# mprib/caliscope

Hardware: AMD Instinct MI355X
Metric: observations/sec per LM iteration (higher is better)
Workload: dtype f64; 1 GPU; cfg4: 64 cams / 2000000 obs in total (200000 points / 2000000 obs on rank 0), extrinsics-only BA, linear loss; n_obs_total=2000000, params_per_camera=6, tolerances=ftol=xtol=gtol=1e-8 (reference defaults), sums=FP64 atomics (default)

## Files before the change

### caliscope_amd/build.py

```python

from __future__ import annotations

import os
import shutil
import subprocess
import sys
from pathlib import Path

HERE = Path(__file__).resolve().parent
CSRC = HERE / "csrc"
OUT = HERE / "libcaliscope_ba.so"
SOURCES = [CSRC / "cba_lib.hip", CSRC / "cba_solve.cpp", CSRC / "pose_lib.hip", CSRC / "scale_lib.hip", CSRC / "coverage_lib.hip", CSRC / "vertical_lib.hip", CSRC / "report_lib.hip", CSRC / "trajectory_lib.hip", CSRC / "covariance_lib.hip"]
DEPENDS = [CSRC / "cba_kernels.h", CSRC / "schur_plan.h", CSRC / "host_plan.h", CSRC / "wg_binding.h", CSRC / "ba_math.h", CSRC / "trf_math.h", CSRC / "pnp_math.h", CSRC / "epipolar_math.h", CSRC / "intrinsic_math.h", CSRC / "frame_select_math.h", CSRC / "scale_math.h", CSRC / "coverage_math.h", CSRC / "vertical_math.h", CSRC / "report_math.h", CSRC / "trajectory_math.h", CSRC / "covariance_math.h", CSRC / "device_call.h",
           HERE.parent / "include" / "caliscope_ba.h", HERE.parent / "include" / "caliscope_pose.h", HERE.parent / "include" / "caliscope_coverage.h", HERE.parent / "include" / "caliscope_vertical.h", HERE.parent / "include" / "caliscope_report.h", HERE.parent / "include" / "caliscope_trajectory.h", HERE.parent / "include" / "caliscope" / "uncertainty.h"]
ARCH = "gfx950"


def hipcc_path() -> str:
    for cand in (os.environ.get("HIPCC"), shutil.which("hipcc"), "/opt/rocm/bin/hipcc"):
        if cand and Path(cand).exists():
            return cand
    raise RuntimeError("hipcc not found (expected /opt/rocm/bin/hipcc)")


def needs_build() -> bool:
    if not OUT.exists():
        return True
    t = OUT.stat().st_mtime
    return any(p.stat().st_mtime > t for p in SOURCES + DEPENDS)


def source_digest() -> str:
    import hashlib

    h = hashlib.sha256()
    for path in sorted(SOURCES + DEPENDS, key=lambda q: q.name):
        h.update(path.name.encode())
        h.update(path.read_bytes())
    return h.hexdigest()


def built_digest(path: Path = OUT) -> str | None:
    import re

    m = re.search(rb"CBA_SOURCE_DIGEST=([0-9a-f]{64})", path.read_bytes())
    return m.group(1).decode() if m else None


def build(force: bool = False, verbose: bool = True) -> Path:
    if not force and not needs_build() and built_digest() == source_digest():
        return OUT
    cmd = [
        hipcc_path(), f"--offload-arch={ARCH}", "-O3", "-std=c++17", "-shared", "-fPIC", "-munsafe-fp-atomics",
        "-Wall", "-Wno-unused-function", f'-DCBA_SOURCE_DIGEST="{source_digest()}"', *map(str, SOURCES), "-o", str(OUT), "-pthread", "-lrccl",
        "-lrocprofiler-sdk-roctx",
    ]
    if verbose:
        print("[caliscope_amd.build]", " ".join(cmd), flush=True)
    subprocess.run(cmd, check=True, cwd=str(CSRC))
    return OUT


if __name__ == "__main__":
    build(force="--force" in sys.argv)
    print(OUT)
```

### caliscope_amd/csrc/cba_kernels.h

```cpp
#pragma once
#include <hip/hip_runtime.h>

#include "ba_math.h"
#include "trf_math.h"
#include "wg_binding.h"

namespace cba {

constexpr int BLOCK = 256;
constexpr int CHUNK = 256;
constexpr int WAVE = 64;

struct VecLayout {
  int ncp;
  int ncp_pad;
  int P;
  int Ppad;
  __host__ __device__ long total() const { return (long)ncp_pad + 3L * Ppad; }
};

__device__ __forceinline__ double wave_sum(double v) {
#pragma unroll
  for (int o = WAVE / 2; o > 0; o >>= 1) v += __shfl_down(v, o, WAVE);
  return v;
}
__device__ __forceinline__ double wave_max(double v) {
#pragma unroll
  for (int o = WAVE / 2; o > 0; o >>= 1) v = fmax(v, __shfl_down(v, o, WAVE));
  return v;
}
#ifdef CBA_PROFILING
constexpr int STAMP_SLOTS = 96, STAMP_BLOCKS = 1024, STAMP_WAVES = 16, STAMP_ROW = 1 + STAMP_WAVES;
__device__ long long* g_cba_stamps = nullptr;
struct StampScope {
  long long* row;
  __device__ __forceinline__ explicit StampScope(int slot) : row(nullptr) {
    long long* base = g_cba_stamps;
    const int b = (int)(blockIdx.y * gridDim.x + blockIdx.x);
    if (base && slot < STAMP_SLOTS && b < STAMP_BLOCKS) {
      row = base + ((long)slot * STAMP_BLOCKS + b) * STAMP_ROW;
      if (threadIdx.x == 0 && threadIdx.y == 0) row[0] = wall_clock64();
    }
  }
  __device__ __forceinline__ ~StampScope() {
    const int t = (int)(threadIdx.y * blockDim.x + threadIdx.x);
    if (row && (t & (WAVE - 1)) == 0 && t / WAVE < STAMP_WAVES) row[1 + t / WAVE] = wall_clock64();
  }
};
#define CBA_STAMP(slot) StampScope cba_stamp_scope_(slot)
#else
#define CBA_STAMP(slot) ((void)0)
#endif
enum StampId { ST_TPREP = 0, ST_PAIRS, ST_REG_REDUCE, ST_FINALIZE, ST_CHOL_APPLY, ST_BACKSUB, ST_STEP_CAM, ST_BUILD, ST_REDUCE_PUB, ST_SCALE_LIN, ST_JV,
               ST_SMALL_SOLVE, ST_CHOL_STEP  };

__device__ __forceinline__ double block_sum(double v, double* sh) {
  v = wave_sum(v);
  const int lane = threadIdx.x & (WAVE - 1), w = threadIdx.x / WAVE;
  __syncthreads();
  if (lane == 0) sh[w] = v;
  __syncthreads();
  double r = 0.0;
  if (threadIdx.x == 0)
    for (int i = 0; i < BLOCK / WAVE; ++i) r += sh[i];
  return r;
}
__device__ __forceinline__ double block_max(double v, double* sh) {
  v = wave_max(v);
  const int lane = threadIdx.x & (WAVE - 1), w = threadIdx.x / WAVE;
  __syncthreads();
  if (lane == 0) sh[w] = v;
  __syncthreads();
  double r = 0.0;
  if (threadIdx.x == 0)
    for (int i = 0; i < BLOCK / WAVE; ++i) r = fmax(r, sh[i]);
  return r;
}

__device__ __forceinline__ void lds_add(double* addr, double v) { unsafeAtomicAdd(addr, v); }

constexpr int CAMTAB_LIVE = 36;
constexpr int CAMTAB_LDS = CAMTAB_LIVE + 1;
struct ObsRec { double u, v; int cam, pt; };
__device__ __forceinline__ ObsRec load_obs(const double* __restrict__ obs_u, const double* __restrict__ obs_v,
                                           const int* __restrict__ obs_cam, const int* __restrict__ obs_pt, int i) {
  ObsRec r;
  r.u = obs_u[i]; r.v = obs_v[i]; r.cam = obs_cam[i]; r.pt = obs_pt[i];
  return r;
}

__device__ __forceinline__ void stage_camtab(double* sh_tab, const double* tab, int n_cams) {
  for (int i = threadIdx.x; i < n_cams * CAMTAB_LIVE; i += BLOCK)
    sh_tab[(i / CAMTAB_LIVE) * CAMTAB_LDS + (i % CAMTAB_LIVE)] = tab[(i / CAMTAB_LIVE) * CAMTAB_DOUBLES + (i % CAMTAB_LIVE)];
}
__device__ __forceinline__ const CamTab& cam_at(const double* sh_tab, int cam) {
  return *reinterpret_cast<const CamTab*>(sh_tab + cam * CAMTAB_LDS);
}
template <bool CAMG>
__device__ __forceinline__ const CamTab& cam_of(const double* sh_tab, const double* __restrict__ tab, int cam) {
  if constexpr (CAMG) return *reinterpret_cast<const CamTab*>(tab + (long)cam * CAMTAB_DOUBLES);
  else return cam_at(sh_tab, cam);
}

__global__ void k_cam_prep(const double* __restrict__ xvec, const double* __restrict__ cam_const,
                           const int* __restrict__ cam_model, const int* __restrict__ cam_np,
                           const int* __restrict__ cam_off, int n_cams, double* __restrict__ tab) {
  const int c = blockIdx.x * blockDim.x + threadIdx.x;
  if (c >= n_cams) return;
  double xc[MAX_NC];
  const int np = cam_np[c];
  for (int i = 0; i < MAX_NC; ++i) xc[i] = (i < np) ? xvec[cam_off[c] + i] : 0.0;
  CamTab t;
  cam_prepare(xc, cam_const + c * CAM_CONST_STRIDE, cam_model[c], np, &t, cam_off[c]);
  const double* src = reinterpret_cast<const double*>(&t);
  for (int i = 0; i < CAMTAB_DOUBLES; ++i) tab[c * CAMTAB_DOUBLES + i] = src[i];
}

__global__ void __launch_bounds__(BLOCK)
k_begin(const double* __restrict__ x0, double* __restrict__ x, double* __restrict__ x_new, double* __restrict__ sinv, double* __restrict__ cam_diag,
        int* __restrict__ flags, long total, int ncp_pad, const double* __restrict__ cam_const, const int* __restrict__ cam_model,
        const int* __restrict__ cam_np, const int* __restrict__ cam_off, int n_cams, double* __restrict__ tab) {
  const long t0 = (long)blockIdx.x * blockDim.x + threadIdx.x;
  for (long i = t0; i < total; i += (long)gridDim.x * blockDim.x) {
    const double v = x0[i];
    x[i] = v;
    if (x_new) x_new[i] = v;
    sinv[i] = 1.0;
    if (i < ncp_pad) cam_diag[i] = 0.0;
    if (i < 4) flags[i] = 0;
  }
  if (t0 < n_cams) {
    const int c = (int)t0;
    double xc[MAX_NC];
    const int np = cam_np[c];
    for (int i = 0; i < MAX_NC; ++i) xc[i] = (i < np) ? x0[cam_off[c] + i] : 0.0;
    CamTab t;
    cam_prepare(xc, cam_const + c * CAM_CONST_STRIDE, cam_model[c], np, &t, cam_off[c]);
    const double* src = reinterpret_cast<const double*>(&t);
    for (int i = 0; i < CAMTAB_DOUBLES; ++i) tab[c * CAMTAB_DOUBLES + i] = src[i];
  }
}

template <bool WRITE_R, bool CAMG = false>
__global__ void __launch_bounds__(BLOCK)
k_cost(const double* __restrict__ obs_u, const double* __restrict__ obs_v, const int* __restrict__ obs_cam,
       const int* __restrict__ obs_pt, long n_obs, const double* __restrict__ xvec, VecLayout lay,
       const double* __restrict__ tab, int n_cams, int loss, double f_scale, double* __restrict__ partial,
       int* __restrict__ flags, double* __restrict__ r_out, const int* __restrict__ order) {
  extern __shared__ __attribute__((aligned(16))) double sh[];
  double* sh_tab = sh;
  double* sh_red = sh + (CAMG ? 0 : n_cams * CAMTAB_LDS);
  if (!CAMG) stage_camtab(sh_tab, tab, n_cams);
  __syncthreads();
  const double* px = xvec + lay.ncp_pad;
  double acc = 0.0;
  bool bad = false;
  struct Rec { int cam, pt; double u, v; long o; };
  const long stride = (long)gridDim.x * BLOCK, last = n_obs - 1;
// ... 1724 lines not shown
    v = -sum;
  } else {
    v = -Sacc[(long)row * ncp + col];
  }
  if (same_cam) v += Upacked[param_cam[row] * UP::STRIDE + UP::idx(param_loc[row], param_loc[col])];
  if (row == col) v += lam * sinv[row] * sinv[row] + cam_diag[row];
  return v;
}
template <int NC>
__global__ void __launch_bounds__(256)
k_schur_finalize(const double* __restrict__ Sacc, const double* __restrict__ bacc,
                 const double* __restrict__ Upacked, const double* __restrict__ gvec,
                 const double* __restrict__ sinv, const int* __restrict__ param_cam,
                 const int* __restrict__ param_loc, int ncp, double lam, const double* __restrict__ lam_dev,
                 const double* __restrict__ cam_diag, double* __restrict__ S, double* __restrict__ rhs,
                 double* __restrict__ W, int ldw, const double* __restrict__ red = nullptr, int g = 0, long tile_elems = 0,
                 const int* __restrict__ group_cam_begin = nullptr, int b_width = 0) {
  CBA_STAMP(ST_FINALIZE);
  if (lam_dev) lam = *lam_dev;
  const long t = (long)blockIdx.x * blockDim.x + threadIdx.x;
  if (t >= (long)ncp * ncp) return;
  const int row = (int)(t / ncp), col = (int)(t % ncp);
  if (col < row) return;
  const double v = schur_entry<NC>(row, col, Sacc, Upacked, sinv, param_cam, param_loc, ncp, lam, cam_diag, red, g, tile_elems, group_cam_begin);
  if (row == col) {
    const double rv = -gvec[row] + b_entry(bacc, b_width, row);
    rhs[row] = rv;
    W[(long)ncp * ldw + row] = rv;
  }
  S[(long)row * ncp + col] = v;
  S[(long)col * ncp + row] = v;
  W[(long)row * ldw + col] = v;
  W[(long)col * ldw + row] = v;
}

template <int NC>
__global__ void __launch_bounds__(64 * REG_REDUCE_Y_MAX)
k_reg_finalize(TilePlan tp, const int* __restrict__ tile_wg_begin, const double* __restrict__ partial, const int* __restrict__ cam_off,
               const int* __restrict__ cam_np, int ncp, int n_tiles, int G, int ysplit, int fold_x, int rhs_x, int tile_x,
               const double* __restrict__ partial_b, int b_rows, int b_width,
               const double* __restrict__ Upacked, const double* __restrict__ gvec, const double* __restrict__ sinv, double lam,
               const double* __restrict__ lam_dev, const double* __restrict__ cam_diag, double* __restrict__ S, double* __restrict__ rhs,
               double* __restrict__ W, int ldw) {
  CBA_STAMP(ST_REG_REDUCE);
  using UP = UPack<NC>;
  constexpr int YM = REG_REDUCE_Y_MAX;
  __shared__ double sh[YM][64];
  const int tx = threadIdx.x, ty = threadIdx.y;
  const int g = tp.g, bsz = NC * NC;
  auto put = [&](int row, int col, double v) {
    S[(long)row * ncp + col] = v; S[(long)col * ncp + row] = v;
    W[(long)row * ldw + col] = v; W[(long)col * ldw + row] = v;
  };
  const int bid = (int)blockIdx.x;
  if (bid >= G * fold_x && bid < G * fold_x + rhs_x) {
    const int j = (bid - G * fold_x) * 64 + tx;
    sh[ty][tx] = (j < b_width) ? strided_sum(partial_b + j, b_width, 0, b_rows, ty, YM) : 0.0;
    __syncthreads();
    if (ty == 0 && j < ncp) {
      double tot = 0.0;
#pragma unroll
      for (int y = 0; y < YM; ++y) tot += sh[y][tx];
      const double rv = -gvec[j] + tot;
      rhs[j] = rv;
      W[(long)ncp * ldw + j] = rv;
    }
    return;
  }
  if (bid < G * fold_x) {
    if (lam_dev) lam = *lam_dev;
    const int ga = bid / fold_x, bx = bid % fold_x;
    const int t = ga * G - ga * (ga - 1) / 2;
    const int ca0 = tp.group_cam_begin[ga], na = tp.group_cam_begin[ga + 1] - ca0;
    const int q = bx * 64 + tx;
    const int cl = q / bsz, r = (q % bsz) / NC, c = (q % bsz) % NC;
    const bool live = q < g * bsz && cl < na && c >= r && c < cam_np[ca0 + min(cl, max(na - 1, 0))];
    constexpr int HMAX = kSchurRegMaxGroupK * (kSchurRegMaxGroupK + 1) / 2;
    __shared__ int sh_hoff[3][HMAX];
    const int cl_first = (bx * 64) / bsz;
    for (int e = ty * 64 + tx; e < 3 * HMAX; e += 64 * YM) {
      const int cam_l = cl_first + e / HMAX, h = e % HMAX, k = cam_l + h * max(na, 1);
      int off = 0;
      if (cam_l < na && k < g * (g + 1) / 2) {
        int li = (int)((sqrtf(8.0f * k + 1.0f) - 1.0f) * 0.5f);
        while (li * (li + 1) / 2 > k) --li;
        while ((li + 1) * (li + 2) / 2 <= k) ++li;
        off = (li * g + (k - li * (li + 1) / 2)) * bsz;
      }
      sh_hoff[e / HMAX][h] = off;
    }
    __syncthreads();
    double a[8] = {0.0, 0.0, 0.0, 0.0, 0.0, 0.0, 0.0, 0.0};
    const int w0 = tile_wg_begin[t] * tp.rep, R = tile_wg_begin[t + 1] * tp.rep - w0;
    if (live && R > 0) {
      const int H = (g * (g + 1) / 2 - cl + na - 1) / na;
      const int* hoff = sh_hoff[cl - cl_first];
      const double* base = partial + (long)w0 * tp.tile_elems + r * NC + c;
      int h = ty / R, w = ty % R;
      auto next = [&]() {
        const double* ptr = base + (long)w * tp.tile_elems + hoff[min(h, H - 1)];
        w += YM;
        while (w >= R) { w -= R; ++h; }
        return ptr;
      };
      const int total = H * R;
      int m = ty;
      for (; m + 7 * YM < total; m += 8 * YM) {
        const double* ptr[8];
#pragma unroll
        for (int q = 0; q < 8; ++q) ptr[q] = next();
#pragma unroll
        for (int q = 0; q < 8; ++q) a[q] += *ptr[q];
      }
      for (; m < total; m += YM) a[0] += *next();
    }
    sh[ty][tx] = ((a[0] + a[1]) + (a[2] + a[3])) + ((a[4] + a[5]) + (a[6] + a[7]));
    __syncthreads();
    if (ty != 0 || !live) return;
    double tot = 0.0;
#pragma unroll
    for (int y = 0; y < YM; ++y) tot += sh[y][tx];
    const int cam = ca0 + cl, row = cam_off[cam] + r, col = cam_off[cam] + c;
    double v = Upacked[cam * UP::STRIDE + UP::idx(r, c)] - tot;
    if (r == c) v += lam * sinv[row] * sinv[row] + cam_diag[row];
    put(row, col, v);
    return;
  }
  const int t = (bid - G * fold_x - rhs_x) / tile_x, bx = (bid - G * fold_x - rhs_x) % tile_x;
  const int ga = tp.tile_a[t], gb = tp.tile_b[t];
  const int ca0 = tp.group_cam_begin[ga], na = tp.group_cam_begin[ga + 1] - ca0;
  const int cb0 = tp.group_cam_begin[gb], nb = tp.group_cam_begin[gb + 1] - cb0;
  const int per = YM / ysplit, sub = ty / ysplit, yy = ty % ysplit;
  const int e = (bx * per + sub) * 64 + tx;
  const int w0 = tile_wg_begin[t] * tp.rep, w1 = tile_wg_begin[t + 1] * tp.rep;
  int row = -1, col = -1;
  if (e < g * g * bsz) {
    const int beta = e / bsz, rc = e % bsz;
    const int li = beta / g, lj = beta % g, r = rc / NC, c = rc % NC;
    if (!(ga == gb && lj <= li) && li < na && lj < nb && r < cam_np[ca0 + li] && c < cam_np[cb0 + lj]) {
      row = cam_off[ca0 + li] + r; col = cam_off[cb0 + lj] + c;
    }
  }
  sh[ty][tx] = (row >= 0) ? strided_sum(partial + e, tp.tile_elems, w0, w1, yy, ysplit) : 0.0;
  __syncthreads();
  if (yy != 0 || row < 0) return;
  double tot = 0.0;
  for (int y = 0; y < ysplit; y += 4) tot += (sh[ty + y][tx] + sh[ty + y + 1][tx]) + (sh[ty + y + 2][tx] + sh[ty + y + 3][tx]);
  put(row, col, -tot);
}

typedef double v4f64 __attribute__((ext_vector_type(4)));
constexpr int CHOL_THREADS = 512;

__device__ __forceinline__ void chol_rank_nb(const double* __restrict__ A, int rcA, const double* __restrict__ B, int rcB,
                                             int ldw, double (*red)[16][17], int wv, int lane) {
  if (wv >= 4) return;
  const int ti = wv >> 1, tj = wv & 1, lr = lane & 15, kq = 4 * (lane >> 4);
  const double* pa = A + (long)min(ti * 16 + lr, rcA - 1) * ldw + kq;
  const double* pb = B + (long)min(tj * 16 + lr, rcB - 1) * ldw + kq;
  double2 a[NB / 16][2], b[NB / 16][2];
#pragma unroll
  for (int s = 0; s < NB / 16; ++s)
#pragma unroll
    for (int h = 0; h < 2; ++h) {
      a[s][h] = *reinterpret_cast<const double2*>(pa + 16 * s + 2 * h);
      b[s][h] = *reinterpret_cast<const double2*>(pb + 16 * s + 2 * h);
    }
  v4f64 c = {0.0, 0.0, 0.0, 0.0};
#pragma unroll
  for (int s = 0; s < NB / 16; ++s)
#pragma unroll
    for (int h = 0; h < 2; ++h) {
      c = __builtin_amdgcn_mfma_f64_16x16x4f64(a[s][h].x, b[s][h].x, c, 0, 0, 0);
      c = __builtin_amdgcn_mfma_f64_16x16x4f64(a[s][h].y, b[s][h].y, c, 0, 0, 0);
    }
#pragma unroll
  for (int r = 0; r < 4; ++r) red[wv][(lane >> 4) + 4 * r][lr] = c[r];
}

__global__ void __launch_bounds__(CHOL_THREADS)
k_chol_step(double* __restrict__ W, int n, int ldw, int k, int* __restrict__ flags, long long* __restrict__ trace, double* __restrict__ Xinv,
            double* __restrict__ Tinv = nullptr) {
  CBA_STAMP(ST_CHOL_STEP + k + 1);
  __shared__ double sh_red[4][16][17];
  __shared__ double sh_U[NB][NB + 1], sh_X[NB][NB + 1], sh_D[2 * NB][NB + 1];
  __shared__ __attribute__((aligned(16))) double sh_L[NB][NB + 2];
  const int tid = threadIdx.x, wv = tid >> 6, lane = tid & 63;
  const int nbk = (n + NB - 1) / NB;
  constexpr int EPT = NB * NB / CHOL_THREADS, ISTEP = CHOL_THREADS / NB;
  const int j = tid & 31, i0 = tid >> 5;
  const int n_panel = (k < 0) ? 1 : nbk - k;
  const int n_trailing = (k < 1) ? 0 : (nbk - k - 1) * (nbk - k) / 2;

  if ((int)blockIdx.x >= n_panel + n_trailing) {
    const int t2 = blockIdx.x - n_panel - n_trailing;
    const int bi = k + t2 / k, bj = t2 % k, m = k - 1;
    const int ri = bi * NB, rci = min(NB, n - ri), rj = bj * NB, rcj = min(NB, n - rj);
    double* Tb = Tinv + (long)rj * ldw + ri;
    double old[EPT];
#pragma unroll
    for (int h = 0; h < EPT; ++h) {
      const int i = i0 + h * ISTEP;
      old[h] = (m != bj && i < rcj && j < rci) ? Tb[(long)i * ldw + j] : 0.0;
    }
    chol_rank_nb(Tinv + (long)rj * ldw + m * NB, rcj, W + (long)ri * ldw + m * NB, rci, ldw, sh_red, wv, lane);
    __syncthreads();
    if (bi != k) {
#pragma unroll
      for (int h = 0; h < EPT; ++h) {
        const int i = i0 + h * ISTEP;
        if (i < rcj && j < rci) Tb[(long)i * ldw + j] = old[h] + sh_red[(i >> 4) * 2 + (j >> 4)][i & 15][j & 15];
      }
      return;
    }
#pragma unroll
    for (int h = 0; h < EPT; ++h) {
      const int i = i0 + h * ISTEP;
      sh_U[i][j] = (i < rcj && j < rci) ? old[h] + sh_red[(i >> 4) * 2 + (j >> 4)][i & 15][j & 15] : 0.0;
      sh_L[i][j] = Xinv[(long)k * NB * NB + i * NB + j];
    }
    __syncthreads();
    if (wv < 4) {
      const int ti = wv >> 1, tj = wv & 1;
      v4f64 c = {0.0, 0.0, 0.0, 0.0};
#pragma unroll
      for (int t = 0; t < NB / 4; ++t) {
        const int q = 4 * t + (lane >> 4);
        c = __builtin_amdgcn_mfma_f64_16x16x4f64(sh_U[ti * 16 + (lane & 15)][q], sh_L[tj * 16 + (lane & 15)][q], c, 0, 0, 0);
      }
#pragma unroll
      for (int r = 0; r < 4; ++r) {
        const int i = ti * 16 + (lane >> 4) + 4 * r, jj = tj * 16 + (lane & 15);
        if (i < rcj && jj < rci) Tb[(long)i * ldw + jj] = -c[r];
      }
    }
    return;
  }

  if ((int)blockIdx.x >= n_panel) {
    int t = blockIdx.x - n_panel, bj = k + 1;
    while (t >= nbk - bj) { t -= nbk - bj; ++bj; }
    const int bi = bj + 1 + t;
    const int ri = (bi < nbk) ? bi * NB : n, rci = (bi < nbk) ? min(NB, n - ri) : 1;
    const int rj = bj * NB, rcj = min(NB, n - rj);
    const int m0 = (k - 1) * NB;
    double* Wi = W + (long)ri * ldw;
    double w_ij[EPT];
#pragma unroll
    for (int h = 0; h < EPT; ++h) {
      const int i = i0 + h * ISTEP;
      w_ij[h] = (i < rci && j < rcj) ? Wi[(long)i * ldw + rj + j] : 0.0;
    }
    chol_rank_nb(Wi + m0, rci, W + (long)rj * ldw + m0, rcj, ldw, sh_red, wv, lane);
    __syncthreads();
#pragma unroll
    for (int h = 0; h < EPT; ++h) {
      const int i = i0 + h * ISTEP;
      if (i < rci && j < rcj) Wi[(long)i * ldw + rj + j] = w_ij[h] - sh_red[(i >> 4) * 2 + (j >> 4)][i & 15][j & 15];
    }
    return;
  }

  const int b = k + 1 + blockIdx.x;
  const int rb = (b < nbk) ? b * NB : n;
  const int rc = (b < nbk) ? min(NB, n - rb) : 1;
  const bool has_diag = b < nbk;
  double* Wb = W + (long)rb * ldw;
  const bool stamp = trace != nullptr && blockIdx.x == 0 && tid == 0;
#define CHOL_STAMP(ph) do { if (stamp) trace[(k + 1) * 8 + (ph)] = wall_clock64(); } while (0)
  CHOL_STAMP(0);

  double d_ij[EPT], m_ij[EPT], l_ij[EPT];
#pragma unroll
  for (int h = 0; h < EPT; ++h) {
    const int i = i0 + h * ISTEP;
    d_ij[h] = (has_diag && i < rc && j < rc) ? Wb[(long)i * ldw + rb + j] : (i == j ? 1.0 : 0.0);
  }
  if (k < 0) {
#pragma unroll
    for (int h = 0; h < EPT; ++h) sh_D[i0 + h * ISTEP][j] = d_ij[h];
  } else {
    const int k0 = k * NB, nbp = min(NB, n - k0);
#pragma unroll
    for (int h = 0; h < EPT; ++h) {
      const int i = i0 + h * ISTEP;
      m_ij[h] = (i < rc && j < nbp) ? Wb[(long)i * ldw + k0 + j] : 0.0;
      l_ij[h] = Xinv[(long)k * NB * NB + i * NB + j];
    }

    CHOL_STAMP(1);
    if (k >= 1) chol_rank_nb(Wb + (k0 - NB), rc, W + (long)k0 * ldw + (k0 - NB), nbp, ldw, sh_red, wv, lane);
    __syncthreads();
    CHOL_STAMP(2);
#pragma unroll
    for (int h = 0; h < EPT; ++h) {
      const int i = i0 + h * ISTEP;
      const double upd = (k >= 1) ? sh_red[(i >> 4) * 2 + (j >> 4)][i & 15][j & 15] : 0.0;
      sh_U[i][j] = m_ij[h] - upd;
      sh_L[i][j] = l_ij[h];
    }
    __syncthreads();
    CHOL_STAMP(3);
    if (wv < 4) {
      const int ti = wv >> 1, tj = wv & 1;
      v4f64 c = {0.0, 0.0, 0.0, 0.0};
#pragma unroll
      for (int t = 0; t < NB / 4; ++t) {
        const int q = 4 * t + (lane >> 4);
        c = __builtin_amdgcn_mfma_f64_16x16x4f64(sh_U[ti * 16 + (lane & 15)][q], sh_L[tj * 16 + (lane & 15)][q], c, 0, 0, 0);
      }
#pragma unroll
      for (int r = 0; r < 4; ++r) {
        const int i = ti * 16 + (lane >> 4) + 4 * r, jj = tj * 16 + (lane & 15);
        sh_X[i][jj] = (jj < nbp && i < rc) ? c[r] : 0.0;
      }
    }
    __syncthreads();
#pragma unroll
    for (int h = 0; h < EPT; ++h) {
      const int i = i0 + h * ISTEP;
      if (i < rc && j < nbp) Wb[(long)i * ldw + k0 + j] = sh_X[i][j];
    }
    CHOL_STAMP(4);
    if (!has_diag) return;
    if (wv < 4) {
      const int ti = wv >> 1, tj = wv & 1;
      v4f64 c = {0.0, 0.0, 0.0, 0.0};
#pragma unroll
      for (int t = 0; t < NB / 4; ++t) {
        const int q = 4 * t + (lane >> 4);
        c = __builtin_amdgcn_mfma_f64_16x16x4f64(sh_X[ti * 16 + (lane & 15)][q], sh_X[tj * 16 + (lane & 15)][q], c, 0, 0, 0);
      }
#pragma unroll
      for (int r = 0; r < 4; ++r) sh_red[wv][(lane >> 4) + 4 * r][lane & 15] = c[r];
    }
    __syncthreads();
#pragma unroll
    for (int h = 0; h < EPT; ++h) {
      const int i = i0 + h * ISTEP;
      const double d_new = d_ij[h] - sh_red[(i >> 4) * 2 + (j >> 4)][i & 15][j & 15];
      if (b != k + 1) {
        if (i < rc && j < rc) Wb[(long)i * ldw + rb + j] = d_new;
      } else {
        sh_D[i][j] = (i < rc && j < rc) ? d_new : (i == j ? 1.0 : 0.0);
      }
    }
    if (b != k + 1) return;
  }
  __syncthreads();
  CHOL_STAMP(5);
  if (tid < WAVE) chol_factor_block(sh_D, rc, flags);
  __syncthreads();
  chol_factor_store(sh_D, rc, Wb + rb, ldw, Xinv + (long)(k + 1) * NB * NB, tid, CHOL_THREADS, Tinv ? Tinv + (long)rb * ldw + rb : nullptr);
  CHOL_STAMP(6);
#undef CHOL_STAMP
}

constexpr int SMALL_N = 96;
constexpr int SMALL_THREADS = 512;
constexpr int SMALL_LD = SMALL_N + 1;
template <int NC>
__global__ void __launch_bounds__(SMALL_THREADS)
k_small_solve(const double* __restrict__ Sacc, const double* __restrict__ bacc, const double* __restrict__ Upacked, const double* __restrict__ gvec,
              const double* __restrict__ sinv, const int* __restrict__ param_cam, const int* __restrict__ param_loc, int n, double lam,
              const double* __restrict__ lam_dev, const double* __restrict__ cam_diag, double* __restrict__ S, double* __restrict__ rhs,
              const double* __restrict__ red, int g, long tile_elems, const int* __restrict__ group_cam_begin, int* __restrict__ flags,
              double* __restrict__ out, int b_width) {
  CBA_STAMP(ST_SMALL_SOLVE);
  using UP = UPack<NC>;
  extern __shared__ __attribute__((aligned(16))) double sh[];
  double (*W)[SMALL_LD] = reinterpret_cast<double (*)[SMALL_LD]>(sh);
  double (*D)[NB + 1] = reinterpret_cast<double (*)[NB + 1]>(sh + (SMALL_N + 1) * SMALL_LD);
  double (*X)[NB][NB + 1] = reinterpret_cast<double (*)[NB][NB + 1]>(&D[2 * NB][0]);
  double* y = &X[(SMALL_N + NB - 1) / NB][0][0];
  if (lam_dev) lam = *lam_dev;
  const int tid = threadIdx.x, nbk = (n + NB - 1) / NB;
  int* pc = reinterpret_cast<int*>(y + SMALL_N);
  int* pl = pc + SMALL_N;
  for (int i = tid; i < n; i += SMALL_THREADS) {
    pc[i] = param_cam[i]; pl[i] = param_loc[i];
    const double rv = -gvec[i] + b_entry(bacc, b_width, i);
    rhs[i] = rv;
    W[n][i] = rv;
  }
  __syncthreads();
  for (int base = tid; base < n * n; base += 4 * SMALL_THREADS) {
    double v4[4];
    int r4[4], c4[4];
#pragma unroll
    for (int u = 0; u < 4; ++u) {
      const int t = base + u * SMALL_THREADS;
      const int row = min(t, n * n - 1) / n, col = min(t, n * n - 1) % n;
      const bool live = t < n * n && col > row && pc[row] != pc[col];
      r4[u] = live ? row : -1; c4[u] = col;
      v4[u] = -Sacc[(long)row * n + col];
    }
#pragma unroll
    for (int u = 0; u < 4; ++u) {
      if (r4[u] < 0) continue;
      S[(long)r4[u] * n + c4[u]] = v4[u]; S[(long)c4[u] * n + r4[u]] = v4[u];
      W[r4[u]][c4[u]] = v4[u]; W[c4[u]][r4[u]] = v4[u];
    }
  }
  for (int q = tid; q < n * NC; q += SMALL_THREADS) {
    const int row = q / NC, col = row - pl[row] + q % NC;
    if (col < row || col >= n || pc[col] != pc[row]) continue;
    const int cam = pc[row];
    double v;
    if (red) {
      const int ga = cam / g, ca0 = group_cam_begin[ga], na = group_cam_begin[ga + 1] - ca0;
      const double* src = red + (long)ga * tile_elems + pl[row] * NC + pl[col];
      double sum = 0.0;
      for (int k = cam - ca0; k < g * (g + 1) / 2; k += na) {
        int li = (int)((sqrtf(8.0f * k + 1.0f) - 1.0f) * 0.5f);
        while (li * (li + 1) / 2 > k) --li;
        while ((li + 1) * (li + 2) / 2 <= k) ++li;
        const int lj = k - li * (li + 1) / 2;
        sum += src[(long)(li * g + lj) * (NC * NC)];
      }
      v = -sum;
    } else {
      v = -Sacc[(long)row * n + col];
    }
    v += Upacked[cam * UP::STRIDE + UP::idx(pl[row], pl[col])];
    if (row == col) v += lam * sinv[row] * sinv[row] + cam_diag[row];
    S[(long)row * n + col] = v; S[(long)col * n + row] = v;
    W[row][col] = v; W[col][row] = v;
  }
  __syncthreads();
  for (int k = 0; k < nbk; ++k) {
    const int k0 = k * NB, nb = min(NB, n - k0);
    for (int e = tid; e < NB * NB; e += SMALL_THREADS) {
      const int i = e / NB, j = e % NB;
      D[i][j] = (i < nb && j < nb) ? W[k0 + max(i, j)][k0 + min(i, j)] : (i == j ? 1.0 : 0.0);
    }
    __syncthreads();
    if (tid < WAVE) chol_factor_block(D, nb, flags);
    __syncthreads();
    for (int e = tid; e < NB * NB; e += SMALL_THREADS) {
      const int i = e / NB, j = e % NB;
      if (i < nb && j <= i) W[k0 + i][k0 + j] = D[i][j];
      X[k][i][j] = D[NB + j][i];
    }
    __syncthreads();
    const int r_lo = k0 + nb, n_rows = n + 1 - r_lo;
    double acc4[(SMALL_N + 1) * NB / SMALL_THREADS + 1];
    {
      int q = 0;
      for (int e = tid; e < n_rows * NB; e += SMALL_THREADS, ++q) {
        const int r = r_lo + e / NB, j = e % NB;
        double a = 0.0;
        if (j < nb)
          for (int t = 0; t <= j; ++t) a = fma(W[r][k0 + t], X[k][j][t], a);
        acc4[q] = a;
      }
    }
    __syncthreads();
    {
      int q = 0;
      for (int e = tid; e < n_rows * NB; e += SMALL_THREADS, ++q) {
        const int r = r_lo + e / NB, j = e % NB;
        if (j < nb) W[r][k0 + j] = acc4[q];
      }
    }
    __syncthreads();
    const int m = n - r_lo;
    for (int e = tid; e < (m + 1) * m; e += SMALL_THREADS) {
      const int i = r_lo + e / m, j = r_lo + e % m;
      if (j > i) continue;
      double a = W[i][j];
      for (int t = 0; t < nb; ++t) a = fma(-W[i][k0 + t], W[j][k0 + t], a);
      W[i][j] = a;
    }
    __syncthreads();
  }
  for (int i = tid; i < n; i += SMALL_THREADS) y[i] = W[n][i];
  __syncthreads();
  for (int k = nbk - 1; k >= 0; --k) {
    const int k0 = k * NB, nb = min(NB, n - k0);
    double xv = 0.0;
    if (tid < nb) {
      for (int t = tid; t < nb; ++t) xv = fma(X[k][t][tid], y[k0 + t], xv);
    }
    __syncthreads();
    if (tid < nb) { y[k0 + tid] = xv; out[k0 + tid] = xv; }
    __syncthreads();
    for (int i = tid; i < k0; i += SMALL_THREADS) {
      double a = y[i];
      for (int t = 0; t < nb; ++t) a = fma(-W[k0 + t][i], y[k0 + t], a);
      y[i] = a;
    }
    __syncthreads();
  }
}

constexpr int APPLY_THREADS = 512;
__global__ void __launch_bounds__(APPLY_THREADS)
k_chol_apply(const double* __restrict__ Tinv, const double* __restrict__ W, int n, int ldw, double* __restrict__ out) {
  CBA_STAMP(ST_CHOL_APPLY);
  extern __shared__ __attribute__((aligned(16))) double y[];
  const int tid = threadIdx.x;
  for (int i = tid; i < n; i += APPLY_THREADS) y[i] = W[(long)n * ldw + i];
  __syncthreads();
  const int r = tid >> 4, cl = tid & 15, row = blockIdx.x * NB + r;
// ... 1451 lines not shown
```

### caliscope_amd/csrc/cba_lib.hip

```cpp
#include <hip/hip_runtime.h>

#include <algorithm>
#include <atomic>
#include <chrono>
#include <cmath>
#include <condition_variable>
#include <cstdarg>
#include <cstdio>
#include <cstdlib>
#include <cstring>
#include <map>
#include <mutex>
#include <shared_mutex>
#include <memory>
#include <string>
#include <type_traits>
#include <thread>
#include <utility>
#include <vector>

#include <rccl/rccl.h>
#include <rocprofiler-sdk-roctx/roctx.h>

#include "../../include/caliscope_ba.h"
#include "cba_kernels.h"
#include "schur_plan.h"
#include "host_plan.h"
#include "wg_binding.h"

using namespace cba;

#ifndef CBA_SOURCE_DIGEST
#define CBA_SOURCE_DIGEST "unknown"
#endif
extern "C" __attribute__((used, visibility("hidden"))) const char cba_source_digest_marker[] = "CBA_SOURCE_DIGEST=" CBA_SOURCE_DIGEST;

static thread_local std::string g_last_error;

static int fail(int code, const char* fmt, ...) {
  char buf[1024];
  va_list ap;
  va_start(ap, fmt);
  vsnprintf(buf, sizeof(buf), fmt, ap);
  va_end(ap);
  g_last_error = buf;
  return code;
}

#define HIPCHK(expr)                                                                                   \
  do {                                                                                                 \
    hipError_t _e = (expr);                                                                            \
    if (_e != hipSuccess)                                                                              \
      return fail(CBA_ERR_HIP, "%s failed: %s (%s:%d)", #expr, hipGetErrorString(_e), __FILE__, __LINE__); \
  } while (0)

enum TimerId {
  T_CAM_PREP = 0, T_COST, T_BUILD, T_BUILD_REDUCE, T_SCALE_SCALARS, T_JV, T_SCHUR, T_SCHUR_REDUCE, T_CHOLESKY,
  T_BACKSUB, T_VECTOR, T_SCHUR_PAIRS, T_EXCHANGE, T_COUNT
};
static const char* kTimerNames[T_COUNT] = {
    "cam_prep", "cost", "build", "build_reduce", "scale_scalars", "jv", "schur", "schur_reduce_finalize",
    "cholesky_solve", "backsub", "vector_ops", "schur_pairs", "exchange"};

struct EventPair { hipEvent_t a, b; };
struct cba_group;

constexpr int JV_ROWS = 2048, CON_ROWS = 1024, PARTIAL4_ROWS = JV_ROWS + CON_ROWS;

struct cba_problem {
  int device = 0;
  hipStream_t stream = nullptr;
  int C = 0, P = 0, ncp = 0, nct = 6;
  long N = 0;
  VecLayout lay{};
  int n_chunks = 0, grid = 0, max_obs_per_point = 0;
  int G = 1, gsz = 1, n_tiles = 1, n_tile_chunks = 0, tile_grid = 0;
  int cus = 256;
  double plan_lane_util = 0.0;
  long tile_stream_len = 0, n_pairs = 0;
  TilePlan tp{};
  int* tile_wg_begin = nullptr;
  int loss = 0;
  double f_scale = 1.0;
  long device_bytes = 0;
  double *obs_u = nullptr, *obs_v = nullptr;
  int *obs_cam = nullptr, *obs_pt = nullptr, *pt_start = nullptr, *chunk_start = nullptr, *order = nullptr;
  int* chunk_pts = nullptr;
  double* cam_const = nullptr;
  int *cam_model = nullptr, *cam_np = nullptr, *cam_off = nullptr, *param_cam = nullptr, *param_loc = nullptr;
  double *tab = nullptr, *tab_new = nullptr;
  double *x0 = nullptr, *x = nullptr, *x_new = nullptr, *g = nullptr, *s = nullptr, *sinv = nullptr, *v1 = nullptr, *v2 = nullptr;
  double *V = nullptr, *Upacked = nullptr;
  double *partial = nullptr, *partial4 = nullptr, *partial1 = nullptr;
  long partial_width = 0;
  bool want_chol_trace = false;
  long long* chol_trace = nullptr;
  int ldw = 0;
  double *Sacc = nullptr, *S = nullptr, *Lbuf = nullptr, *rhs = nullptr, *red = nullptr, *Trec = nullptr, *partial_b = nullptr;
  CsPlan cs{};
  bool tab_global = false;
  int det_m = 0;
  DetPlan det{nullptr, nullptr};
  double* tri = nullptr;
  double* Xinv = nullptr;
  double* Tinv = nullptr;
  bool fuse_reg_finalize = true;
  double* scal = nullptr;
  double* xbuf = nullptr;
  double *sinv_state_c = nullptr, *cam_diag = nullptr, *cam_over1 = nullptr, *cam_over2 = nullptr;
  bool cam_scaled = false, cam_state_saved = false;
  double *fz = nullptr, *V2 = nullptr, *g2 = nullptr, *U2 = nullptr, *partial4b = nullptr;
  bool eval_only = false;
  bool peer_needs_primitives = false;
  bool have_build = false;
  bool trial_built = false;
  bool cost_pending = false;
  double cost_x = 0.0;
  double trial_cost = 0.0;
  int grid_backsub = 1;
  int jv_grid = 0;
  bool has_fragments = false;
  bool backsub_rec = false;
  int n_heavy = 0; int* heavy_pts = nullptr; int* heavy_frag = nullptr; double* heavy_W = nullptr;
  std::vector<int> h_heavy_pts;
  ConPlan con{};
  int con_grid = 0;
  int n_con_orphan = 0; int* con_orphan = nullptr;
  int* flags = nullptr;
  double* h_scal = nullptr;
  int* h_flags = nullptr;
  double* d_hscal = nullptr;
  double *h_cam = nullptr, *d_hcam = nullptr;
  double *h_bcam = nullptr, *d_hbcam = nullptr;
  double *lb_dev = nullptr, *ub_dev = nullptr, *sinv_state_c2 = nullptr, *cam_diag2 = nullptr;
  bool bounds_on = false;
  unsigned long long publish_seq = 0;
  bool spin_wait = true;
  int* d_hflags = nullptr;
  bool first_scale = true;
  double* sinv2 = nullptr;
  bool spec_enqueued = false, spec_valid = false;
  int spec_rows_jv = 0;
  bool spec_skip = true, tol_set = false, last_trial_hint = false;
  double ftol = 0.0, xtol = 0.0;
  int* spec_word = nullptr;
  bool spec_jv_enqueued = false;
  bool spec_jv_dropped = false;
  bool spec_scale_ready = false;
  long spec_jv_skipped = 0;
  unsigned long long gnorm_seq = 0;
  bool gnorm_mailed = false;
  bool lf_pending = false;
  LinFin lf{};
  bool have_x0 = false;
  std::vector<int> h_tile_wg_begin;
  struct PlanTask* plan_task = nullptr;
  int reg_reduce_y = 4;
  int plan_max_blocks = 0;
  size_t partial_capacity = 0;
  bool plan_is_cheap = false;
  int plan_error = 0;
  bool schur_clock = false;
  long long* stamps = nullptr;
  bool begun = false, linearized = false, stepped = false, have_trial = false;
  double gh_sq = 0.0;
  std::vector<int> h_cam_off, h_cam_np;
  double* h_vec = nullptr;
  size_t h_vec_doubles = 0;
  hipEvent_t h_vec_sent = nullptr;
  bool h_vec_in_flight = false;
  bool timers_on = false;
  std::vector<EventPair> pending[T_COUNT];
  std::vector<EventPair> free_events;
  double t_ms[T_COUNT] = {0};
  long t_calls[T_COUNT] = {0};
  std::vector<void*> allocs;
  std::vector<size_t> alloc_bytes;
  size_t mail_doubles = 0;
  char* arena_cur = nullptr; size_t arena_left = 0, arena_next = (size_t)4 << 20;
  char* up_stage = nullptr; size_t up_cap = 0, up_used = 0;
  std::atomic<ncclComm_t> comm{nullptr};
  std::atomic<bool> comm_aborted{false};
  cba_group* group = nullptr;
  int rank = 0, world = 1;
  unsigned long long group_generation = 0;
  bool sharded() const { return comm.load() != nullptr || group != nullptr || comm_aborted.load(); }
  bool small_solve_on = true;
  bool one_workgroup_solve() const { return ncp <= SMALL_N && small_solve_on && !sharded() && !chol_trace; }
};

constexpr size_t kPoolChunk = (size_t)4 << 20;
constexpr size_t kPoolKeep = 4;
constexpr size_t kPoolStagingMax = (size_t)8 << 20;
struct DevicePool {
  std::vector<void*> chunks;
  std::vector<hipStream_t> streams;
  std::vector<std::pair<double*, size_t>> mail;
  std::vector<std::pair<double*, size_t>> staging;
  std::vector<char*> upstage;
};
constexpr size_t kUpStage = (size_t)256 << 10, kUpStageMax = (size_t)64 << 10;
static std::mutex g_pool_mu;
static std::map<int, DevicePool> g_pool;

template <typename T>
static int dev_alloc(cba_problem* p, T** out, size_t count) {
  const size_t bytes = (std::max<size_t>(count, 1) * sizeof(T) + 255) & ~(size_t)255;
  if (bytes > p->arena_left) {
    const size_t chunk = std::max(bytes, p->arena_next);
    void* ptr = nullptr;
    if (chunk == kPoolChunk) {
      std::lock_guard<std::mutex> lock(g_pool_mu);
      DevicePool& pool = g_pool[p->device];
      if (!pool.chunks.empty()) { ptr = pool.chunks.back(); pool.chunks.pop_back(); }
    }
    if (!ptr) HIPCHK(hipMalloc(&ptr, chunk));
    p->allocs.push_back(ptr);
    p->alloc_bytes.push_back(chunk);
    if (bytes >= p->arena_next) {
      p->device_bytes += (long)bytes;
      *out = static_cast<T*>(ptr);
      return CBA_OK;
    }
    p->arena_cur = static_cast<char*>(ptr);
    p->arena_left = chunk;
    p->arena_next = std::min<size_t>(p->arena_next * 2, (size_t)256 << 20);
  }
  *out = reinterpret_cast<T*>(p->arena_cur);
  p->arena_cur += bytes;
  p->arena_left -= bytes;
  p->device_bytes += (long)bytes;
  return CBA_OK;
}
template <typename T>
static int dev_upload(cba_problem* p, T** out, const T* h, size_t count) {
  int rc = dev_alloc(p, out, count);
  if (rc) return rc;
  const size_t bytes = count * sizeof(T);
  if (bytes && p->up_stage && p->stream && bytes <= kUpStageMax && p->up_used + bytes <= p->up_cap) {
    std::memcpy(p->up_stage + p->up_used, h, bytes);
    HIPCHK(hipMemcpyAsync(*out, p->up_stage + p->up_used, bytes, hipMemcpyHostToDevice, p->stream));
    p->up_used += (bytes + 63) & ~(size_t)63;
  } else if (bytes) {
    HIPCHK(hipMemcpy(*out, h, bytes, hipMemcpyHostToDevice));
  }
  return CBA_OK;
}
template <typename T, typename V>
static int dev_upload(cba_problem* p, T** out, const V& h) {
  static_assert(std::is_same<typename std::remove_cv<typename std::remove_pointer<decltype(h.data())>::type>::type, T>::value, "element type");
  return dev_upload(p, out, h.data(), h.size());
}
template <typename T>
static int dev_zeros(cba_problem* p, T** out, size_t count) {
  int rc = dev_alloc(p, out, count);
  if (rc) return rc;
  HIPCHK(hipMemsetAsync(*out, 0, count * sizeof(T), p->stream));
  return CBA_OK;
// ... 716 lines not shown
        p->grid_backsub = std::max(1, std::min(p->n_chunks, p->cus * resident_per_cu(k_backsub_rec<NC, true>, lds_backsub_rec<NC>(p), 2)));
    }
  }
  {
    int per_cu = p->tab_global ? resident_per_cu(k_jv<NC, 1, true>, lds_jv(p, 1), 2) : resident_per_cu(k_jv<NC, 1>, lds_jv(p, 1), 2);
    if (const char* e = std::getenv("CBA_JV_WGS")) per_cu = std::max(1, std::min(std::atoi(e), 8));
    p->jv_grid = (int)std::max<long>(1, std::min<long>((p->N + BLOCK - 1) / BLOCK, (long)p->cus * per_cu));
    p->jv_grid = std::min(p->jv_grid, JV_ROWS);
  }
  if (p->n_heavy && (rc = allow_lds(k_heavy_schur<NC>, (size_t)p->ncp * 3 * sizeof(double) + (size_t)p->ncp * sizeof(int)))) return rc;
  if ((rc = allow_lds(k_chol_apply, (size_t)p->ncp * 8))) return rc;
  if ((rc = allow_lds(k_step_cam, (size_t)p->lay.ncp_pad * 8))) return rc;
  if (p->one_workgroup_solve() && (rc = allow_lds(k_small_solve<NC>, kSmallSolveLds))) return rc;
  return CBA_OK;
}


static void start_plan_task(cba_problem* p, const cba_options* opt, int n_cus, const int* hcam, const int* hps) {
  constexpr long kTwoStageObs = 500000;
  const char* plan_env = std::getenv("CBA_PLAN");
  bool plan_two_stage = p->N >= kTwoStageObs;
  if (plan_env && std::strcmp(plan_env, "swap") == 0) plan_two_stage = true;
  if (plan_env && (std::strcmp(plan_env, "full") == 0 || std::strcmp(plan_env, "cheap") == 0)) plan_two_stage = false;
  if ((opt && opt->deterministic) || p->schur_clock) plan_two_stage = false;
  Reg2Params prm = (p->nct == 9) ? reg2_params<9, Reg3Cfg<9>>(p) : reg2_params<6, Reg3Cfg<6>>(p);
  if (plan_env) prm.cheap = std::strcmp(plan_env, "cheap") == 0;
  p->plan_task = new PlanTask();
  {
    const int cus0 = n_cus > 0 ? n_cus : 256;
    const size_t tile_lds = (p->nct == 9) ? Reg3Cfg<9>::LDS_BYTES : Reg3Cfg<6>::LDS_BYTES;
    const int per_cu = std::min(std::max<int>(1, (int)((160 * 1024) / tile_lds)), (p->nct == 9) ? RegCfg<9>::PER_CU : RegCfg<6>::PER_CU);
    const int mb0 = (opt && opt->max_blocks > 0) ? opt->max_blocks : 2 * cus0;
    p->plan_max_blocks = std::min(cus0 * per_cu, std::max(mb0, cus0));
  }
  p->plan_task->start(prm, hcam, hps, plan_two_stage, p);
}

static int open_stream_and_mailbox(cba_problem* p, const MailLayout& mail) {
  {
    std::lock_guard<std::mutex> lock(g_pool_mu);
    DevicePool& pool = g_pool[p->device];
    if (!pool.streams.empty()) { p->stream = pool.streams.back(); pool.streams.pop_back(); }
    for (size_t i = 0; i < pool.mail.size(); ++i)
      if (pool.mail[i].second >= mail.total) {
        p->h_scal = pool.mail[i].first; p->mail_doubles = pool.mail[i].second;
        pool.mail.erase(pool.mail.begin() + (long)i);
        break;
      }
  }
  if (!p->stream) HIPCHK(hipStreamCreateWithFlags(&p->stream, hipStreamNonBlocking));
  if (!p->h_scal) {
    p->mail_doubles = std::max<size_t>(mail.total, MailLayout(96).total);
    HIPCHK(hipHostMalloc((void**)&p->h_scal, p->mail_doubles * sizeof(double), hipHostMallocMapped));
  }
  HIPCHK(hipHostGetDevicePointer((void**)&p->d_hscal, p->h_scal, 0));
  p->h_cam = p->h_scal + mail.cam; p->d_hcam = p->d_hscal + mail.cam;
  p->h_flags = reinterpret_cast<int*>(p->h_scal + mail.flags); p->d_hflags = reinterpret_cast<int*>(p->d_hscal + mail.flags);
  p->h_bcam = p->h_scal + mail.bcam; p->d_hbcam = p->d_hscal + mail.bcam;
  std::memset(p->h_scal, 0, mail.total * sizeof(double));
  return CBA_OK;
}

#define TRYS(e) do { const int rc_ = (e); if (rc_) return rc_; } while (0)

static int upload_observations(cba_problem* p, const double* obs_uv, const SortedObs& obs, const PointTables& tabs) {
  TRYS(dev_upload(p, &p->obs_cam, obs.cam)); TRYS(dev_upload(p, &p->obs_pt, obs.pt));
  TRYS(dev_upload(p, &p->order, obs.order)); TRYS(dev_upload(p, &p->pt_start, tabs.pt_start)); TRYS(dev_upload(p, &p->chunk_start, tabs.chunk_start));
  double* uv_raw = nullptr;
  TRYS(dev_upload(p, &uv_raw, obs_uv, (size_t)2 * p->N)); TRYS(dev_alloc(p, &p->obs_u, (size_t)p->N)); TRYS(dev_alloc(p, &p->obs_v, (size_t)p->N));
  hipLaunchKernelGGL(k_gather_uv, dim3((int)std::min<long>((p->N + 255) / 256, 2048)), dim3(256), 0, p->stream, (const double*)uv_raw, (const int*)p->order, p->N, p->obs_u, p->obs_v);
  return CBA_OK;
}

static int upload_det_plan(cba_problem* p, const HostDetPlan& plan) {
  unsigned char* dperm = nullptr; unsigned short* dcst = nullptr;
  TRYS(dev_upload(p, &dperm, plan.perm)); TRYS(dev_upload(p, &dcst, plan.cst));
  p->det_m = plan.det_m;
  p->det = DetPlan{dperm, dcst};
  return CBA_OK;
}

static int upload_cs_plan(cba_problem* p, const HostCsPlan& plan) {
  double *dcu = nullptr, *dcv = nullptr;
  int *dcc = nullptr, *dcp = nullptr, *dso = nullptr, *dp0 = nullptr, *dnp = nullptr, *dperm = nullptr;
  TRYS(dev_upload(p, &dperm, plan.cperm));
  TRYS(dev_alloc(p, &dcu, (size_t)p->N)); TRYS(dev_alloc(p, &dcv, (size_t)p->N)); TRYS(dev_alloc(p, &dcc, (size_t)p->N)); TRYS(dev_alloc(p, &dcp, (size_t)p->N));
  TRYS(dev_upload(p, &dso, plan.sc_obs)); TRYS(dev_upload(p, &dp0, plan.sc_p0)); TRYS(dev_upload(p, &dnp, plan.sc_np));
  hipLaunchKernelGGL(k_cs_fill, dim3(plan.n_sc), dim3(256), 0, p->stream, (const int*)dperm, (const int*)dso, (const int*)dp0, (const double*)p->obs_u, (const double*)p->obs_v,
                     (const int*)p->obs_cam, (const int*)p->obs_pt, dcu, dcv, dcc, dcp);
  p->cs = CsPlan{dcu, dcv, dcc, dcp, dso, dp0, dnp, plan.n_sc, plan.pmax};
  return CBA_OK;
}

static int upload_cameras(cba_problem* p, const double* cam_const, const CameraLayout& cams, const PointTables& tabs) {
  if (p->n_heavy) {
    TRYS(dev_upload(p, &p->heavy_pts, tabs.heavy)); TRYS(dev_upload(p, &p->heavy_frag, tabs.heavy_frag));
    TRYS(dev_alloc(p, &p->heavy_W, (size_t)p->n_heavy * p->ncp * 3));
  }
  TRYS(dev_upload(p, &p->cam_const, cam_const, (size_t)p->C * 12));
  TRYS(dev_upload(p, &p->cam_model, cams.model)); TRYS(dev_upload(p, &p->cam_np, cams.np)); TRYS(dev_upload(p, &p->cam_off, cams.off));
  TRYS(dev_upload(p, &p->param_cam, cams.param_cam)); TRYS(dev_upload(p, &p->param_loc, cams.param_loc));
  return CBA_OK;
}

static int alloc_vectors(cba_problem* p) {
  TRYS(dev_alloc(p, &p->tab, (size_t)p->C * CAMTAB_DOUBLES)); TRYS(dev_alloc(p, &p->tab_new, (size_t)p->C * CAMTAB_DOUBLES));
  for (double** v : {&p->x0, &p->x, &p->x_new, &p->g, &p->s, &p->sinv, &p->v1, &p->v2, &p->sinv2}) TRYS(dev_zeros(p, v, (size_t)p->lay.total()));
  for (double** v : {&p->sinv_state_c, &p->cam_diag, &p->cam_over1, &p->cam_over2, &p->lb_dev, &p->ub_dev, &p->sinv_state_c2, &p->cam_diag2})
    TRYS(dev_zeros(p, v, (size_t)p->lay.ncp_pad));
  TRYS(dev_zeros(p, &p->V, (size_t)6 * p->lay.Ppad));
  const int ustride = (p->nct == 9) ? UPack<9>::STRIDE : UPack<6>::STRIDE;
  TRYS(dev_alloc(p, &p->Upacked, (size_t)p->C * ustride + 128));
  return CBA_OK;
}

static int install_first_plan(cba_problem* p, bool plan_timing) {
  PlanTask& task = *p->plan_task;
  const auto t_wait = std::chrono::steady_clock::now();
  task.wait_stage(task.two_stage ? 1 : 2);
  if (plan_timing) {
    fprintf(stderr, "  plan: %s took %.3f s on its own threads, started before the uploads; waited %.3f s for it\n", task.two_stage ? "the cheap plan" : "dealt streams and codes",
            task.two_stage ? task.seconds_cheap : task.seconds, std::chrono::duration<double>(std::chrono::steady_clock::now() - t_wait).count());
    const Reg2Plan& made = task.two_stage ? task.cheap : task.plan;
    fprintf(stderr, "  plan: its phases: point runs %.4f s, jobs %.4f s, concatenation %.4f s (%.0f MB)\n", made.seconds_runs, made.seconds_jobs, made.seconds_concat,
            (made.obs.size() + made.codes.size()) * 4e-6);
  }
  if (task.two_stage ? task.rc_cheap : task.rc)
    return fail(CBA_ERR_UNSUPPORTED, "a world point has more observations inside one camera-group tile than a chunk of the pair plan holds (%d records)",
                (p->nct == 9) ? Reg3Cfg<9>::SCHUNK : Reg3Cfg<6>::SCHUNK);
  const int rc = install_reg2_plan(p, task.two_stage ? task.cheap : task.plan, task.prm);
  p->plan_is_cheap = task.two_stage || task.prm.cheap;
  return rc;
}

static int alloc_solver_buffers(cba_problem* p) {
  const int ncp = p->ncp, nct = p->nct;
  const long tot = p->lay.total();
  const int ustride = (nct == 9) ? UPack<9>::STRIDE : UPack<6>::STRIDE;
  const long w_build = (long)p->C * ustride;
  p->partial_width = w_build;
  p->partial_capacity = (size_t)std::max<long>((long)p->grid * w_build, (long)(p->tile_grid + p->tile_grid / 8 + 1) * std::max(p->tp.rep, 1) * p->tp.tile_elems);
  TRYS(dev_alloc(p, &p->partial, p->partial_capacity));
  TRYS(dev_alloc(p, &p->partial4, (size_t)PARTIAL4_ROWS * 4)); TRYS(dev_alloc(p, &p->partial1, (size_t)2048)); TRYS(dev_alloc(p, &p->partial4b, (size_t)2048 * 4));
  TRYS(dev_zeros(p, &p->Sacc, (size_t)ncp * ncp + (size_t)B_SLICES * p->lay.ncp_pad));
  TRYS(dev_alloc(p, &p->tri, (size_t)ncp * (ncp + 1) / 2 + p->lay.ncp_pad));
  if (!p->eval_only) {
    TRYS(dev_alloc(p, &p->red, (size_t)p->G * p->tp.tile_elems));
    TRYS(dev_alloc(p, &p->Trec, (size_t)std::max<long>(p->N, 1) * ((nct == 9) ? SchurRec<9>::HREC : SchurRec<6>::HREC)));
    TRYS(dev_alloc(p, &p->partial_b, (size_t)p->grid * p->lay.ncp_pad));
  }
  TRYS(dev_alloc(p, &p->S, (size_t)ncp * ncp)); p->ldw = (ncp + 3) & ~3;
  if (p->want_chol_trace) TRYS(dev_alloc(p, &p->chol_trace, (size_t)((ncp + NB - 1) / NB + 2) * 8));
  TRYS(dev_alloc(p, &p->Lbuf, (size_t)(ncp + 1) * p->ldw));
  TRYS(dev_alloc(p, &p->Xinv, (size_t)((ncp + NB - 1) / NB + 1) * NB * NB));
  TRYS(dev_zeros(p, &p->Tinv, (size_t)ncp * p->ldw));
  TRYS(dev_alloc(p, &p->rhs, (size_t)p->lay.ncp_pad));
  TRYS(dev_zeros(p, &p->scal, 64)); TRYS(dev_zeros(p, &p->flags, 8)); TRYS(dev_alloc(p, &p->xbuf, 128));
  p->spec_word = p->flags + 4;
  TRYS(dev_alloc(p, &p->fz, 8)); TRYS(dev_zeros(p, &p->V2, (size_t)6 * p->lay.Ppad)); TRYS(dev_zeros(p, &p->g2, (size_t)tot));
  TRYS(dev_alloc(p, &p->U2, (size_t)p->C * ustride + 128));
  return CBA_OK;
}

static int open_staging(cba_problem* p) {
  const size_t tot = (size_t)p->lay.total();
  {
    std::lock_guard<std::mutex> lock(g_pool_mu);
    DevicePool& pool = g_pool[p->device];
    for (size_t i = 0; i < pool.staging.size(); ++i)
      if (pool.staging[i].second >= tot && pool.staging[i].second <= 4 * tot + 4096) {
        p->h_vec = pool.staging[i].first; p->h_vec_doubles = pool.staging[i].second;
        pool.staging.erase(pool.staging.begin() + (long)i);
        break;
      }
  }
  HIPCHK(hipEventCreateWithFlags(&p->h_vec_sent, hipEventDisableTiming));
  if (!p->h_vec) {
    p->h_vec_doubles = tot;
    HIPCHK(hipHostMalloc((void**)&p->h_vec, p->h_vec_doubles * sizeof(double), hipHostMallocDefault));
  }
  return CBA_OK;
}
static int device_synchronize() { HIPCHK(hipDeviceSynchronize()); return CBA_OK; }
#undef TRYS

extern "C" {

int cba_create(const cba_problem_desc* d, const cba_options* opt, cba_problem** out) {
  if (!d || !out) return fail(CBA_ERR_INVALID, "cba_create: null argument");
  *out = nullptr;
  if (const int rc = validate_problem_desc(fail, d)) return rc;
  const double t_enter = std::chrono::duration<double>(std::chrono::steady_clock::now().time_since_epoch()).count();
  int ndev = 0;
  if (hipGetDeviceCount(&ndev) != hipSuccess || ndev <= 0)
    return fail(CBA_ERR_NO_DEVICE, "no HIP device available: the MI355X engine has no CPU fallback");
  int dev = (opt && opt->device_id >= 0) ? opt->device_id : 0;
  if (!(opt && opt->device_id >= 0)) (void)hipGetDevice(&dev);
  if (dev >= ndev) return fail(CBA_ERR_INVALID, "device %d requested, %d available", dev, ndev);
  HIPCHK(hipSetDevice(dev));
  int n_cus = 0;
  if (hipDeviceGetAttribute(&n_cus, hipDeviceAttributeMultiprocessorCount, dev) != hipSuccess) n_cus = 0;

  cba_problem* p = new cba_problem();
  p->device = dev;
  p->C = d->n_cams; p->P = d->n_points; p->N = d->n_obs;
  p->loss = d->loss; p->f_scale = d->f_scale;
  if (const char* e = std::getenv("CBA_REG_FINALIZE")) p->fuse_reg_finalize = e[0] != '0';
  if (const char* e = std::getenv("CBA_SPEC_SKIP")) p->spec_skip = e[0] != '0';
  if (const char* e = std::getenv("CBA_SMALL_SOLVE")) p->small_solve_on = e[0] != '0';
#ifdef CBA_PROFILING
  p->schur_clock = std::getenv("CBA_SCHUR_CLOCK") != nullptr;
  p->want_chol_trace = std::getenv("CBA_CHOL_TRACE") != nullptr;
  if (std::getenv("CBA_STAMPS")) {
    const size_t n = (size_t)STAMP_SLOTS * STAMP_BLOCKS * STAMP_ROW;
    if (hipMalloc((void**)&p->stamps, n * sizeof(long long)) == hipSuccess) {
      (void)hipMemset(p->stamps, 0, n * sizeof(long long));
      (void)hipMemcpyToSymbol(HIP_SYMBOL(g_cba_stamps), &p->stamps, sizeof(p->stamps));
    }
  }
#endif
  int rc = CBA_OK;
#define TRY(e) do { rc = (e); if (rc) { cba_destroy(p); return rc; } } while (0)
  const bool deterministic = opt && opt->deterministic;

  CameraLayout cams;
  TRY(camera_layout(fail, d, cams));
  const int ncp = cams.ncp, nct = cams.nct;
  p->ncp = ncp; p->nct = nct;
  p->h_cam_off = cams.off; p->h_cam_np = cams.np;
  p->lay.ncp = ncp; p->lay.ncp_pad = cams.ncp_pad;
  p->lay.P = p->P; p->lay.Ppad = (p->P + 31) / 32 * 32;

  const bool plan_timing = plan_timing_on();
  auto t_now = []() { return std::chrono::duration<double>(std::chrono::steady_clock::now().time_since_epoch()).count(); };
  double t_mark = t_now();
  auto lap = [&](const char* what) { if (plan_timing) { const double t = t_now(); fprintf(stderr, "cba_create: %-28s %.6f s\n", what, t - t_mark); t_mark = t; } };
  SortedObs obs;
  PointTables tabs;
  {
    HostVec<int64_t> order(p->N), pstart((size_t)p->P + 1), cstart((size_t)p->N + 2);
    const int64_t nch = cba_host_plan(p->P, p->N, d->obs_pt, d->obs_cam, p->C, CHUNK, order.data(), pstart.data(), cstart.data());
    if (nch < 0) TRY((int)nch);
    p->n_chunks = (int)nch;
    lap("sort by point, chunk table");
    gather_sorted(p->N, d->obs_cam, d->obs_pt, order.data(), obs);
    TRY(point_tables(fail, p->P, pstart.data(), nch, cstart.data(), obs.pt.data(), CHUNK, HEAVY_OBS, tabs));
  }
  p->max_obs_per_point = tabs.max_obs_per_point;
  p->n_heavy = (int)tabs.heavy.size();
  p->h_heavy_pts = tabs.heavy;
  p->has_fragments = tabs.has_fragments;
  p->eval_only = opt && opt->evaluation_only != 0;
  choose_schur_groups(p);
  if (!p->eval_only) start_plan_task(p, opt, n_cus, obs.cam.data(), tabs.pt_start.data());

  TRY(open_stream_and_mailbox(p, MailLayout(ncp)));
  const int cus = n_cus > 0 ? n_cus : 256;
  p->cus = cus;
  const int max_blocks = (opt && opt->max_blocks > 0) ? opt->max_blocks : 2 * cus;
  p->grid = std::max(1, std::min(p->n_chunks, max_blocks));
  p->grid_backsub = std::max(1, std::min(p->n_chunks, 2 * cus));
  if (const char* e = std::getenv("CBA_BACKSUB_WGS")) p->grid_backsub = std::max(1, std::min(p->n_chunks, std::min(std::max(std::atoi(e), 1), 8) * cus));

  lap("reorder on host");
  upload_stage_acquire(p);
  TRY(upload_observations(p, d->obs_uv, obs, tabs));
  if (deterministic) {
    HostDetPlan det;
    TRY(det_plan(fail, p->C, nct, p->n_chunks, tabs.chunk_start.data(), obs.cam.data(), CHUNK, DET_ROUND, BLOCK, det));
    TRY(upload_det_plan(p, det));
  }
  TRY(dev_upload(p, &p->chunk_pts, tabs.chunk_pts));
  {
    const char* cs_env = std::getenv("CBA_BUILD_CS");
    HostCsPlan cs;
    cs_plan(!(cs_env && cs_env[0] == '0'), deterministic, p->C, p->N, p->n_chunks, tabs.chunk_start.data(), tabs.chunk_pts.data(), obs.cam.data(), p->grid,
            (nct == 9) ? 4096 : 2048, CHUNK, CS_MAX_PTS, cs);
    if (cs.n_sc) TRY(upload_cs_plan(p, cs));
  }
  TRY(upload_cameras(p, d->cam_const, cams, tabs));
  lap("upload observations");
  TRY(alloc_vectors(p));
  lap("allocate vectors");
  if (nct == 9) TRY(configure_kernels<9>(p)); else TRY(configure_kernels<6>(p));
  lap("reorder, upload, allocate");
  if (!p->eval_only) TRY(install_first_plan(p, plan_timing));
  lap("Schur plan (streams, pairs, upload)");
  TRY(alloc_solver_buffers(p));
  TRY(open_staging(p));
  lap("solver buffers");
  TRY(device_synchronize());
#undef TRY
  upload_stage_release(p);
  lap("device synchronize");
  if (p->plan_task) {
    if (p->plan_task->two_stage) {
      p->plan_task->hcam_keep = std::move(obs.cam);
      p->plan_task->hps_keep = std::move(tabs.pt_start);
    } else {
      drop_plan_task(p);
    }
  }
  if (plan_timing) fprintf(stderr, "cba_create: %.3f s in total\n", t_now() - t_enter);
  *out = p;
  return CBA_OK;
}

static int maybe_swap_plan(cba_problem* p, bool wait);

int cba_plan_wait(cba_problem* p) {
  if (!p) return fail(CBA_ERR_INVALID, "cba_plan_wait: null problem");
  HIPCHK(hipSetDevice(p->device));
  return maybe_swap_plan(p, true);
}

int cba_set_loss(cba_problem* p, int32_t loss, double f_scale) {
  if (!p) return fail(CBA_ERR_INVALID, "cba_set_loss: null problem");
  if (loss < CBA_LOSS_LINEAR || loss > CBA_LOSS_ARCTAN) return fail(CBA_ERR_INVALID, "cba_set_loss: unknown loss %d", loss);
  if (loss != CBA_LOSS_LINEAR && !(f_scale > 0.0)) return fail(CBA_ERR_INVALID, "cba_set_loss: f_scale must be positive");
  p->loss = loss; p->f_scale = f_scale;
  p->have_build = false;
  p->spec_valid = false; p->spec_enqueued = false; p->spec_scale_ready = false;
  return CBA_OK;
}

int cba_get_info(cba_problem* p, cba_info* o) {
  if (!p || !o) return fail(CBA_ERR_INVALID, "null argument");
  o->n_cams = p->C; o->n_points = p->P; o->n_cam_params = p->ncp; o->n_params = p->ncp + 3 * p->P; o->n_obs = p->N;
  o->n_chunks = p->n_chunks; o->grid_blocks = p->grid;
  o->plan_state = !p->plan_is_cheap ? 0 : (p->plan_task ? 1 : 2); o->plan_error = p->plan_error;
  o->schur_groups = p->G; o->schur_tiles = p->n_tiles; o->schur_grid = p->tile_grid; o->schur_stream_len = p->tile_stream_len; o->schur_pairs = p->n_pairs;
  o->max_obs_per_point = p->max_obs_per_point; o->device_bytes = p->device_bytes; o->n_heavy_points = p->n_heavy;
  {
    const bool cs = p->cs.n_sc && !p->det_m && !p->n_heavy;
    const bool camg = cs ? (p->nct == 6 ? build_cs_camg<6>(p) : build_cs_camg<9>(p)) : (p->nct == 6 ? build_camg<6>(p) : build_camg<9>(p));
    const bool uglob = cs && (p->nct == 6 ? build_cs_uglob<6>(p) : build_cs_uglob<9>(p));
    o->build_camg = (camg ? 1 : 0) | (p->tab_global ? 2 : 0) | (cs ? 4 : 0) | (uglob ? 8 : 0) | (p->backsub_rec ? 16 : 0) |
                    (p->con.n_con && p->con.small ? 32 : 0) | (p->one_workgroup_solve() ? 64 : 0);
  }
  o->spec_jv_skipped = p->spec_jv_skipped;
  return CBA_OK;
}

int cba_enable_timers(cba_problem* p, int32_t on) { if (!p) return fail(CBA_ERR_INVALID, "null"); p->timers_on = on != 0; return CBA_OK; }
int cba_reset_timers(cba_problem* p) {
  if (!p) return fail(CBA_ERR_INVALID, "null");
  (void)hipSetDevice(p->device);
  drain_timers(p);
  for (int t = 0; t < T_COUNT; ++t) { p->t_ms[t] = 0; p->t_calls[t] = 0; }
  return CBA_OK;
}
int cba_get_timers(cba_problem* p, double* ms, int64_t* calls) {
  if (!p) return fail(CBA_ERR_INVALID, "null");
  (void)hipSetDevice(p->device);
  drain_timers(p);
  for (int t = 0; t < T_COUNT; ++t) { if (ms) ms[t] = p->t_ms[t]; if (calls) calls[t] = p->t_calls[t]; }
  return CBA_OK;
}

}
// ... 101 lines not shown
      if (pub)
        hipLaunchKernelGGL(k_reduce_rows_pub, dim3((w + 63) / 64 + 1), dim3(64, REDUCE_RY), 0, p->stream, (const double*)p->partial, u_rows, w, Upacked, g,
                           (const int*)p->cam_off, (const int*)p->cam_np, (int)UPack<NC>::STRIDE, (int)UPack<NC>::TRI, *pub);
      else
        hipLaunchKernelGGL(k_reduce_rows, dim3((w + 63) / 64), dim3(64, REDUCE_RY), 0, p->stream, p->partial, u_rows, w, Upacked, g,
                           (const int*)p->cam_off, (const int*)p->cam_np, (int)UPack<NC>::STRIDE, (int)UPack<NC>::TRI);
      return CBA_OK;
    }
    hipLaunchKernelGGL(k_reduce_rows, dim3((w + 63) / 64), dim3(64, REDUCE_RY), 0, p->stream, p->partial, u_rows, w, Upacked,
                       (double*)nullptr, (const int*)nullptr, (const int*)nullptr, 1, 0);
    int rho_rows = p->grid;
    if (p->con.n_con) {
      HIPCHK(hipMemsetAsync(p->con.cdiag, 0, (size_t)3 * p->lay.Ppad * sizeof(double), p->stream));
      if (p->n_con_orphan)
        hipLaunchKernelGGL(k_zero_heavy, dim3((p->n_con_orphan + 63) / 64), dim3(64), 0, p->stream, (const int*)p->con_orphan, p->n_con_orphan, p->lay,
                           g + p->lay.ncp_pad, 3, (double*)nullptr, 0);
      hipLaunchKernelGGL(k_con_eval<true>, dim3(p->con_grid), dim3(BLOCK), 0, p->stream, p->con, xvec, p->lay, p->loss, p->f_scale, g,
                         p->partial1 + p->grid, p->flags, (double*)nullptr);
      rho_rows += p->con_grid;
    }
    hipLaunchKernelGGL(k_reduce_narrow<false>, dim3(1), dim3(BLOCK), 0, p->stream, p->partial1, rho_rows, 1, p->scal + cost_slot);
    if (defer_exchange) return CBA_OK;
    int rc = allreduce_sum(p, Upacked, (size_t)w);
    if (rc) return rc;
    hipLaunchKernelGGL((k_unpack_camera_grad<NC>), dim3((p->C * NC + 255) / 256), dim3(256), 0, p->stream, Upacked,
                       p->cam_off, p->cam_np, p->C, g);
  }
  return CBA_OK;
}

template <int NC>
static int run_build(cba_problem* p) { return run_build_into<NC>(p, p->x, p->tab, p->V, p->g, p->Upacked, 8, nullptr, false, false, 3); }

template <int NC>
static int run_jv(cba_problem* p, int nv, int* rows_out = nullptr, const double* xvec = nullptr, const double* tab = nullptr, const SpecSkip& skip = SpecSkip{}) {
  ScopedTimer t(p, T_JV);
  if (!xvec) { xvec = p->x; tab = p->tab; }
  const int grid = nv == 1 ? p->jv_grid : (int)std::min<long>((p->N + BLOCK - 1) / BLOCK, 1024);
  const int con_rows = p->con.n_con ? p->con_grid : 0;
  if (grid + con_rows > PARTIAL4_ROWS)
    return fail(CBA_ERR_UNSUPPORTED, "run_jv: %d rows of k_jv and %d of k_con_jv exceed the %d rows of partial4", grid, con_rows, PARTIAL4_ROWS);
  auto launch_jv = [&](auto kernel) {
    hipLaunchKernelGGL(kernel, dim3(grid), dim3(BLOCK), lds_jv(p, nv), p->stream, p->obs_u, p->obs_v, p->obs_cam, p->obs_pt,
                       p->N, xvec, p->lay, tab, p->cam_off, p->C, p->loss, p->f_scale, p->v1, p->v2, p->partial4, skip);
  };
  if (nv == 1) { if (p->tab_global) launch_jv(k_jv<NC, 1, true>); else launch_jv(k_jv<NC, 1>); }
  else { if (p->tab_global) launch_jv(k_jv<NC, 2, true>); else launch_jv(k_jv<NC, 2>); }
  int rows = grid;
  if (con_rows) {
    if (nv == 1) hipLaunchKernelGGL(k_con_jv<1>, dim3(p->con_grid), dim3(BLOCK), 0, p->stream, p->con, p->lay, p->v1, p->v2, p->partial4 + 4 * grid);
    else hipLaunchKernelGGL(k_con_jv<2>, dim3(p->con_grid), dim3(BLOCK), 0, p->stream, p->con, p->lay, p->v1, p->v2, p->partial4 + 4 * grid);
    rows += con_rows;
  }
  if (rows_out) { *rows_out = rows; return CBA_OK; }
  hipLaunchKernelGGL(k_reduce_narrow<false>, dim3(1), dim3(BLOCK), 0, p->stream, p->partial4, rows, 4, p->scal + 12);
  return CBA_OK;
}

template <int NC>
static int run_lin_chain(cba_problem* p, bool scalars = true, bool compact = false, double radius = 0.0, bool defer_finish = false) {
  RoctxRange range("cba:linearize");
  p->spec_scale_ready = false; p->gnorm_mailed = false;
  if (!p->have_build) {
    int rcb = run_build<NC>(p);
    if (rcb) return rcb;
    p->cost_pending = true;
    p->have_build = true;
    p->spec_valid = false;
  }
  if (compact && p->spec_valid) {
    p->spec_valid = false;
    if (defer_finish) {
      p->lf = LinFin{p->partial4b, p->partial1, p->partial4, vec_grid(p->lay.total()), p->spec_rows_jv, radius, p->scal, p->fz};
      p->lf_pending = true;
      return CBA_OK;
    }
    ScopedTimer t(p, T_SCALE_SCALARS);
    hipLaunchKernelGGL(k_lin_finish, dim3(1), dim3(BLOCK), 0, p->stream, p->partial4b, p->partial1, vec_grid(p->lay.total()), p->partial4, p->spec_rows_jv, radius,
                       p->scal, p->fz);
    return CBA_OK;
  }
  p->spec_valid = false;
  const long tot = p->lay.total();
  const int vg = vec_grid(tot);
  const bool bnd = defer_finish && p->bounds_on;
  if (bnd && !p->first_scale && !p->cam_scaled)
    HIPCHK(hipMemcpyAsync(p->sinv_state_c, p->sinv, (size_t)p->lay.ncp_pad * sizeof(double), hipMemcpyDeviceToDevice, p->stream));
  if (p->cam_scaled && !bnd)
    HIPCHK(hipMemcpyAsync(p->sinv, p->sinv_state_c, (size_t)p->lay.ncp_pad * sizeof(double), hipMemcpyDeviceToDevice, p->stream));
  p->cam_state_saved = false;
  {
    ScopedTimer t(p, T_SCALE_SCALARS);
    if (compact) {
      const BoundArgs ba = bnd ? BoundArgs{p->lb_dev, p->ub_dev, p->sinv_state_c, p->sinv_state_c, p->cam_diag} : BoundArgs{};
      if (bnd) p->cam_scaled = true;
      auto launch_sl = [&](auto kernel) {
        hipLaunchKernelGGL(kernel, dim3(vg), dim3(BLOCK), 0, p->stream, p->Upacked, p->V, p->param_cam, p->param_loc, p->lay,
                           p->first_scale ? 1 : 0, p->sinv, p->con.n_con ? (const double*)p->con.cdiag : (const double*)nullptr, p->x, p->g, p->v1,
                           p->partial4b, p->partial1, (const double*)nullptr, ba);
      };
      if (bnd) launch_sl(k_scale_lin<NC, true>); else launch_sl(k_scale_lin<NC, false>);
      p->first_scale = false;
      int rows_jv = 0;
      int rcj = run_jv<NC>(p, 1, &rows_jv);
      if (rcj) return rcj;
      if (defer_finish) {
        p->lf = LinFin{p->partial4b, p->partial1, p->partial4, vg, rows_jv, radius, p->scal, p->fz};
        p->lf_pending = true;
        return CBA_OK;
      }
      hipLaunchKernelGGL(k_lin_finish, dim3(1), dim3(BLOCK), 0, p->stream, p->partial4b, p->partial1, vg, p->partial4, rows_jv, radius,
                         p->scal, p->fz);
      return CBA_OK;
    }
    hipLaunchKernelGGL((k_scale_update<NC>), dim3(vg), dim3(BLOCK), 0, p->stream, p->Upacked, p->V, p->param_cam, p->param_loc,
                       p->lay, p->first_scale ? 1 : 0, p->sinv, p->con.n_con ? (const double*)p->con.cdiag : (const double*)nullptr);
    p->first_scale = false;
    if (!scalars) return exchange(p, SLOT(8), false);
    hipLaunchKernelGGL(k_lin_scalars, dim3(vg), dim3(BLOCK), 0, p->stream, p->x, p->g, p->sinv, tot, p->lay.ncp_pad,
                       p->rank == 0 ? 1 : 0, 0, p->v1, p->partial4, p->partial1);
    hipLaunchKernelGGL(k_reduce_narrow<false>, dim3(1), dim3(BLOCK), 0, p->stream, p->partial4, vg, 4, p->scal + 0);
    hipLaunchKernelGGL(k_reduce_narrow<true>, dim3(1), dim3(BLOCK), 0, p->stream, p->partial1, vg, 1, p->scal + 4);
  }
  {
    int rcj = run_jv<NC>(p, 1);
    if (rcj) return rcj;
  }
  return exchange(p, SLOT(0) | SLOT(1) | SLOT(2) | SLOT(3) | SLOT(8) | SLOT(12) | SLOT(13) | SLOT(14) | SLOT(15), true);
}

static void read_linearization(cba_problem* p, cba_linearization* out) {
  if (p->cost_pending) { p->cost_x = p->h_flags[3] ? NAN : 0.5 * p->h_scal[8]; p->cost_pending = false; }
  p->gh_sq = p->h_scal[0];
  out->gh_sq = p->h_scal[0];
  out->x_scaled_norm = std::sqrt(p->h_scal[1]);
  out->x_norm = std::sqrt(p->h_scal[2]);
  out->g_norm_inf = p->h_scal[4];
  out->cost = p->cost_x;
  out->jg_sq = p->h_scal[12];
}

template <int NC>
static int run_linearize(cba_problem* p, cba_linearization* out) {
  int rc = run_lin_chain<NC>(p, true, !p->sharded(), 1.0);
  if (rc) return rc;
  rc = sync_scalars(p, 16);
  if (rc) return rc;
  read_linearization(p, out);
  return CBA_OK;
}

namespace cba {
__attribute__((visibility("hidden"))) void enqueue_chol_factor(double* W, int n, int ldw, int* flags, long long* trace, double* Xinv, double* Tinv,
                                                               hipStream_t stream) {
  const int nbk = (n + NB - 1) / NB;
  for (int k = -1; k < nbk; ++k) {
    const int n_panel = k < 0 ? 1 : nbk - k;
    const int x = nbk - k - 1, n_trailing = k < 1 ? 0 : x * (x + 1) / 2;
    const int n_inverse = (k >= 1) ? (nbk - k) * k : 0;
    hipLaunchKernelGGL(k_chol_step, dim3(n_panel + n_trailing + n_inverse), dim3(CHOL_THREADS), 0, stream, W, n, ldw, k, flags, trace, Xinv, Tinv);
  }
}
}

static int enqueue_cholesky(cba_problem* p) {
  const int n = p->ncp, nbk = (n + NB - 1) / NB;
  enqueue_chol_factor(p->Lbuf, n, p->ldw, p->flags, p->chol_trace, p->Xinv, p->Tinv, p->stream);
  hipLaunchKernelGGL(k_chol_apply, dim3(nbk), dim3(APPLY_THREADS), (size_t)n * 8, p->stream, (const double*)p->Tinv, (const double*)p->Lbuf, n, p->ldw, p->s);
  return CBA_OK;
}

static int run_cholesky(cba_problem* p) {
#ifdef CBA_PROFILING
  if (p->chol_trace) {
    const int nbk = (p->ncp + NB - 1) / NB;
    HIPCHK(hipMemsetAsync(p->chol_trace, 0, (size_t)(nbk + 2) * 8 * sizeof(long long), p->stream));
    int rc = enqueue_cholesky(p);
    if (rc) return rc;
    std::vector<long long> h((size_t)(nbk + 2) * 8);
    HIPCHK(hipMemcpyAsync(h.data(), p->chol_trace, h.size() * sizeof(long long), hipMemcpyDeviceToHost, p->stream));
    HIPCHK(hipStreamSynchronize(p->stream));
    for (int s = 0; s <= nbk; ++s) {
      fprintf(stderr, "chol step %2d:", s - 1);
      for (int ph = 1; ph < 7; ++ph)
        if (h[s * 8 + ph] && h[s * 8 + ph - 1]) fprintf(stderr, " ph%d %6.2f us", ph, (h[s * 8 + ph] - h[s * 8 + ph - 1]) * 0.01); else if (h[s * 8 + ph]) fprintf(stderr, " ph%d (%6.2f)", ph, (h[s * 8 + ph] - h[s * 8]) * 0.01);
      if (s < nbk && h[(s + 1) * 8] && h[s * 8]) fprintf(stderr, "  | to next step start %6.2f us", (h[(s + 1) * 8] - h[s * 8]) * 0.01);
      fprintf(stderr, "\n");
    }
    return CBA_OK;
  }
#endif
  ScopedTimer t(p, T_CHOLESKY);
  return enqueue_cholesky(p);
}

static int run_step_scalars(cba_problem* p, bool formula_w, bool compact = false) {
  ScopedTimer t(p, T_VECTOR);
  const long tot = p->lay.total();
  const int vg = vec_grid(tot);
  const long first = (p->rank == 0) ? 0 : p->lay.ncp_pad;
  if (compact && first == 0 && tot <= STEP_SMALL_MAX) {
    hipLaunchKernelGGL(k_step_small, dim3(1), dim3(STEP_SMALL_THREADS), 0, p->stream, p->g, p->sinv, p->s, tot, p->scal, (const int*)p->flags, p->fz);
    return CBA_OK;
  }
  hipLaunchKernelGGL(k_step_scalars, dim3(vg), dim3(BLOCK), 0, p->stream, p->g, p->sinv, p->s, tot, first, p->partial4);
  if (compact) {
    hipLaunchKernelGGL(k_step_finish, dim3(1), dim3(BLOCK), 0, p->stream, p->partial4, vg, p->scal, (const int*)p->flags, p->fz);
    return CBA_OK;
  }
  hipLaunchKernelGGL(k_reduce_narrow<false>, dim3(1), dim3(BLOCK), 0, p->stream, p->partial4, vg, 4, p->scal + 16);
  if (formula_w) return exchange(p, SLOT(16) | SLOT(17), false);
  int rcv = allreduce_sum(p, p->scal + 16, 2);
  if (rcv) return rcv;
  hipLaunchKernelGGL(k_w_scalar, dim3(vg), dim3(BLOCK), 0, p->stream, p->g, p->sinv, p->s, tot, first, p->scal + 17, p->gh_sq,
                     (const double*)nullptr, p->partial1);
  hipLaunchKernelGGL(k_reduce_narrow<false>, dim3(1), dim3(BLOCK), 0, p->stream, p->partial1, vg, 1, p->scal + 20);
  return exchange(p, SLOT(20), false);
}

static int maybe_swap_plan(cba_problem* p, bool wait) {
  PlanTask* task = p->plan_task;
  if (!task) return CBA_OK;
  if (wait) task->wait_stage(2);
  if (task->stage.load(std::memory_order_acquire) < 2) return CBA_OK;
  int rc = CBA_OK;
  if (task->rc != 0 && task->two_stage) {
    p->plan_error = task->rc;
    fprintf(stderr, "caliscope_ba: the balanced Schur plan could not be built (error %d, %.3f s on its thread): the handle keeps the quick plan\n", task->rc, task->seconds);
    if (wait) rc = fail(task->rc, "cba_plan_wait: the balanced Schur plan could not be built in the background (error %d); the handle keeps the quick plan", task->rc);
  }
  if (task->rc == 0) {
    const size_t need = (size_t)task->install.tile_grid * std::max(task->install.tp.rep, 1) * task->install.tp.tile_elems;
    if (need > p->partial_capacity) {
      rc = dev_alloc(p, &p->partial, need);
      if (!rc) p->partial_capacity = need;
    }
    if (!rc) {
      apply_install(p, task->install);
      p->plan_is_cheap = false;
      if (plan_timing_on()) fprintf(stderr, "  plan: the dealt plan (%.3f s on its own threads, upload included) swapped in\n", task->seconds);
    }
  }
  drop_plan_task(p);
  return rc;
}

#ifdef CBA_PROFILING
template <int NC>
static int run_pairs_clocked(cba_problem* p) {
  if constexpr (NC != 6) return fail(CBA_ERR_UNSUPPORTED, "CBA_SCHUR_CLOCK: six-parameter cameras only");
  else {
    const int nw = Reg3Cfg<6>::NWAVES;
    const size_t n = (size_t)p->tile_grid * nw * 8;
    long long* d = nullptr;
    if (hipMalloc((void**)&d, n * sizeof(long long)) != hipSuccess) return fail(CBA_ERR_HIP, "debug buffer");
    (void)hipMemsetAsync(d, 0, n * sizeof(long long), p->stream);
    if (raise_lds_ceiling((const void*)k_schur_reg3_clk<6, 1, 2>, Reg3Cfg<6>::LDS_BYTES)) return CBA_ERR_HIP;
    hipLaunchKernelGGL((k_schur_reg3_clk<6, 1, 2>), dim3(p->tile_grid), dim3(Reg3Cfg<6>::LAUNCH_THREADS), Reg3Cfg<6>::LDS_BYTES, p->stream, p->tp, p->Trec, p->partial, d, (const double*)p->tab);
    std::vector<long long> h(n);
    (void)hipMemcpyAsync(h.data(), d, n * sizeof(long long), hipMemcpyDeviceToHost, p->stream);
    (void)hipStreamSynchronize(p->stream);
    (void)hipFree(d);
    static const char* names[4] = {"wait for loads", "barrier", "issue", "pairs"};
    auto report = [&](const char* who, auto pick) {
      double sum[8] = {0}, tmax = 0.0;
      size_t waves = 0;
      for (size_t w = 0; w < n / 8; ++w) {
        if (!h[w * 8 + 4] || !pick(w / nw)) continue;
        ++waves;
        for (int k = 0; k < 7; ++k) sum[k] += (double)h[w * 8 + k];
        tmax = std::max(tmax, (double)h[w * 8 + 6]);
      }
      const double wv = (double)std::max<size_t>(waves, 1);
      fprintf(stderr, "%s phases, mean clocks per wave (%zu waves, %.1f trips, %.1f pair iterations each):", who, waves, sum[4] / wv, sum[5] / wv);
      for (int k = 0; k < 4; ++k) fprintf(stderr, "  %s %.0f", names[k], sum[k] / wv);
      fprintf(stderr, "  | in-loop total %.0f, wave lifetime mean %.0f max %.0f\n", (sum[0] + sum[1] + sum[2] + sum[3]) / wv, sum[6] / wv, tmax);
    };
    report("k_schur_reg3", [](size_t) { return true; });
    return CBA_OK;
  }
}
#endif

template <int NC>
static int run_newton_chain(cba_problem* p, double lam, const double* lam_dev, bool compact = false) {
  const int ncp = p->ncp;
  if (p->plan_task) {
    const int rcs = maybe_swap_plan(p, false);
    if (rcs) return rcs;
  }
  RoctxRange range("cba:damped_step");
  {
    RoctxRange r2("cba:schur");
    ScopedTimer t(p, T_SCHUR);
    {
      const bool linf = p->lf_pending;
      p->lf_pending = false;
      auto launch_tprep = [&](auto kernel) {
        hipLaunchKernelGGL(kernel, dim3(p->grid), dim3(BLOCK), lds_tprep<NC>(p), p->stream, p->obs_u, p->obs_v, p->obs_cam, p->obs_pt,
                           p->chunk_start, p->n_chunks, p->x, p->lay, p->tab, p->cam_off, p->C, p->loss, p->f_scale, lam, lam_dev, p->V, p->g,
                           p->sinv, p->Trec, p->partial_b, p->flags, p->det, linf ? p->lf : LinFin{});
      };
      switch (p->det_m) {
        case 3: launch_tprep(k_tprep<NC, 3>); break;
        case 5: launch_tprep(k_tprep<NC, 5>); break;
        case 8: launch_tprep(k_tprep<NC, 8>); break;
        case 16: { if constexpr (NC == 6) launch_tprep(k_tprep<NC, 16>); } break;
        default:
          if (linf) { if (p->tab_global) launch_tprep(k_tprep<NC, 0, true, true>); else launch_tprep(k_tprep<NC, 0, false, true>); }
          else if (p->tab_global) launch_tprep(k_tprep<NC, 0, true>); else launch_tprep(k_tprep<NC, 0>);
          break;
      }
      ScopedTimer tpairs(p, T_SCHUR_PAIRS);
      constexpr int SP = RegCfg<NC>::SPLIT, MW = RegCfg<NC>::MINW;
#ifdef CBA_PROFILING
      if (p->schur_clock) {
        int rcc = run_pairs_clocked<NC>(p);
        if (rcc) return rcc;
      } else
#endif
      hipLaunchKernelGGL((k_schur_reg3<NC, SP, MW>), dim3(p->tile_grid), dim3(Reg3Cfg<NC>::LAUNCH_THREADS), Reg3Cfg<NC>::LDS_BYTES, p->stream, p->tp, p->Trec, p->partial, (const double*)p->tab);
    }
  }
  bool small_solve = false;
  const bool fold_in_finalize = !p->n_heavy && !p->con.n_con && !p->sharded();
  {
    ScopedTimer t(p, T_SCHUR_REDUCE);
    const bool fused_finalize = fold_in_finalize && !p->one_workgroup_solve() && p->fuse_reg_finalize;
    if (fused_finalize) {
      const int per = REG_REDUCE_Y_MAX / p->reg_reduce_y;
      const int tile_x = (p->gsz * p->gsz * NC * NC + 64 * per - 1) / (64 * per), fold_x = (p->gsz * NC * NC + 63) / 64, rhs_x = (p->lay.ncp_pad + 63) / 64;
      hipLaunchKernelGGL((k_reg_finalize<NC>), dim3(p->G * fold_x + rhs_x + p->n_tiles * tile_x), dim3(64, REG_REDUCE_Y_MAX), 0, p->stream, p->tp, p->tile_wg_begin, p->partial,
                         p->cam_off, p->cam_np, ncp, p->n_tiles, p->G, p->reg_reduce_y, fold_x, rhs_x, tile_x, (const double*)p->partial_b, p->grid, p->lay.ncp_pad, p->Upacked, p->g,
                         p->sinv, lam, lam_dev, p->cam_diag, p->S, p->rhs, p->Lbuf, p->ldw);
    } else {
      hipLaunchKernelGGL(k_reg_reduce, dim3(std::max((p->tp.tile_elems + 63) / 64, (p->lay.ncp_pad + 63) / 64), p->n_tiles + B_SLICES), dim3(64, p->reg_reduce_y), 0,
                         p->stream, p->tp, p->tile_wg_begin, p->partial, p->cam_off, p->cam_np, NC, ncp, p->Sacc, p->red, p->n_tiles,
                         (const double*)p->partial_b, p->grid, p->lay.ncp_pad, p->Sacc + (size_t)ncp * ncp);
// ... 938 lines not shown
```

### caliscope_amd/csrc/covariance_lib.hip

```cpp
#include <hip/hip_runtime.h>

#include <algorithm>
#include <cmath>
#include <string>
#include <vector>

#include "ba_math.h"
#include "covariance_math.h"
#include "device_call.h"

namespace cba {
__attribute__((visibility("hidden"))) void enqueue_chol_factor(double* W, int n, int ldw, int* flags, long long* trace, double* Xinv, double* Tinv,
                                                               hipStream_t stream);
}

using namespace cba;

namespace {

constexpr int NB = 32;
typedef double v4f64 __attribute__((ext_vector_type(4)));
enum CovFlag : int { F_POINT = 0, F_DIAG = 1, F_CHOL = 2, F_TINY = 3, F_WHICH = 4, N_FLAGS = 8 };

__device__ __forceinline__ double wave_sum(double v) {
#pragma unroll
  for (int off = 32; off > 0; off >>= 1) v += __shfl_down(v, off, 64);
  return v;
}

__global__ void __launch_bounds__(COV_BLOCK)
k_unc_cam(int32_t n_cams, const int32_t* __restrict__ cam_model, const int32_t* __restrict__ cam_off, const double* __restrict__ cam_const,
          const double* __restrict__ cam_x, double* __restrict__ tab, double* __restrict__ B) {
  const int32_t c = blockIdx.x * COV_BLOCK + threadIdx.x;
  if (c >= n_cams) return;
  const int32_t off = cam_off[c], np = cam_off[c + 1] - off;
  double xc[MAX_NC];
#pragma unroll
  for (int i = 0; i < MAX_NC; ++i) xc[i] = cam_x[(int64_t)c * MAX_NC + i];
  CamTab t;
  cam_prepare(xc, cam_const + (int64_t)c * CAM_CONST_STRIDE, cam_model[c], np, &t, off);
  const double* src = reinterpret_cast<const double*>(&t);
#pragma unroll
  for (int i = 0; i < CAMTAB_DOUBLES; ++i) tab[(int64_t)c * CAMTAB_DOUBLES + i] = src[i];
  double N[MAX_NC][COV_GAUGE];
  cov_gauge_cam(t, N);
#pragma unroll
  for (int r = 0; r < MAX_NC; ++r)
    if (r < np) {
#pragma unroll
      for (int j = 0; j < COV_GAUGE; ++j) B[(int64_t)(off + r) * COV_GAUGE + j] = N[r][j];
    }
}

__global__ void __launch_bounds__(COV_BLOCK)
k_unc_obs(int64_t n_obs, const int64_t* __restrict__ order, const int32_t* __restrict__ obs_cam, const int32_t* __restrict__ obs_pt,
          const double* __restrict__ obs_uv, const double* __restrict__ tab, const double* __restrict__ points, int loss, double f_scale,
          double* __restrict__ Wblk, double* __restrict__ Vobs, int32_t* __restrict__ cam_sorted, double* __restrict__ U, double* __restrict__ cost) {
  const int64_t i = (int64_t)blockIdx.x * COV_BLOCK + threadIdx.x;
  double rho = 0.0;
  if (i < n_obs) {
    const int64_t o = order[i];
    const int32_t cam = obs_cam[o];
    const int64_t p = obs_pt[o];
    const CamTab& c = reinterpret_cast<const CamTab*>(tab)[cam];
    const double X[3] = {points[3 * p], points[3 * p + 1], points[3 * p + 2]};
    const double uv[2] = {obs_uv[2 * o], obs_uv[2 * o + 1]};
    double A[2][MAX_NC], B[2][3], Wb[3 * MAX_NC], Vo[6];
    rho = cov_obs_jacobian(c, X, uv, loss, f_scale, A, B);
    cov_obs_products(A, B, Wb, Vo);
#pragma unroll
    for (int e = 0; e < 3 * MAX_NC; ++e) Wblk[i * (3 * MAX_NC) + e] = Wb[e];
#pragma unroll
    for (int e = 0; e < 6; ++e) Vobs[i * 6 + e] = Vo[e];
    cam_sorted[i] = cam;
    const bool nine = c.nparams == 9.0;
    double* Uc = U + (int64_t)cam * (MAX_NC * MAX_NC);
#pragma unroll
    for (int r = 0; r < MAX_NC; ++r)
#pragma unroll
      for (int q = r; q < MAX_NC; ++q)
        if (q < 6 || nine) atomicAdd(&Uc[r * MAX_NC + q], A[0][r] * A[0][q] + A[1][r] * A[1][q]);
  }
  rho = wave_sum(rho);
  if ((threadIdx.x & 63) == 0 && rho != 0.0) atomicAdd(cost, 0.5 * rho);
}

__global__ void __launch_bounds__(COV_POINT_THREADS)
k_unc_point(const int64_t* __restrict__ pt_start, const int32_t* __restrict__ cam_sorted, const int32_t* __restrict__ cam_off, int32_t ncp,
            const double* __restrict__ points, const double* __restrict__ Wblk, const double* __restrict__ Vobs, double* __restrict__ Y,
            double* __restrict__ Vinv, double* __restrict__ Zbuf, double* __restrict__ B, double* __restrict__ Sacc, int* __restrict__ flags) {
  __shared__ double sh_vi[9], sh_z[3 * COV_GAUGE];
  const int64_t p = blockIdx.x;
  const int t = threadIdx.x;
  const int64_t s = pt_start[p], k = pt_start[p + 1] - s;
  double V[6] = {0.0, 0.0, 0.0, 0.0, 0.0, 0.0};
  for (int64_t a = 0; a < k; ++a) {
#pragma unroll
    for (int e = 0; e < 6; ++e) V[e] += Vobs[(s + a) * 6 + e];
  }
  double Vi[6];
  if (!cov_point_vinv(V, Vi)) {
    if (t == 0) { flags[F_POINT] = 1; atomicMax(&flags[F_WHICH], (int)p + 1); }
    return;
  }
  const double X[3] = {points[3 * p], points[3 * p + 1], points[3 * p + 2]};
  double Z[3][COV_GAUGE];
  cov_point_z(Vi, X, Z);
  if (t == 0) {
#pragma unroll
    for (int e = 0; e < 6; ++e) Vinv[p * 6 + e] = Vi[e];
#pragma unroll
    for (int a = 0; a < 3; ++a)
#pragma unroll
      for (int b = 0; b < 3; ++b) sh_vi[3 * a + b] = cov_sym3(Vi, a, b);
#pragma unroll
    for (int a = 0; a < 3; ++a)
#pragma unroll
      for (int j = 0; j < COV_GAUGE; ++j) { sh_z[a * COV_GAUGE + j] = Z[a][j]; Zbuf[p * (3 * COV_GAUGE) + a * COV_GAUGE + j] = Z[a][j]; }
  }
  __syncthreads();
  constexpr int WB = 3 * MAX_NC;
  for (int64_t it = t; it < k * WB; it += COV_POINT_THREADS) {
    const int64_t a = it / WB;
    const int e = (int)(it % WB), r = e / 3, q = e % 3;
    const double* w = Wblk + (s + a) * WB + 3 * r;
    Y[(s + a) * WB + e] = w[0] * sh_vi[q] + w[1] * sh_vi[3 + q] + w[2] * sh_vi[6 + q];
  }
  __syncthreads();
  for (int64_t it = t; it < k * (MAX_NC * COV_GAUGE); it += COV_POINT_THREADS) {
    const int64_t a = it / (MAX_NC * COV_GAUGE);
    const int e = (int)(it % (MAX_NC * COV_GAUGE)), r = e / COV_GAUGE, j = e % COV_GAUGE;
    const int32_t cam = cam_sorted[s + a], off = cam_off[cam], np = cam_off[cam + 1] - off;
    if (r >= np) continue;
    const double* w = Wblk + (s + a) * WB + 3 * r;
    atomicAdd(&B[(int64_t)(off + r) * COV_GAUGE + j], -(w[0] * sh_z[j] + w[1] * sh_z[COV_GAUGE + j] + w[2] * sh_z[2 * COV_GAUGE + j]));
  }
  constexpr int BLK = MAX_NC * MAX_NC;
  for (int64_t it = t; it < k * k * BLK; it += COV_POINT_THREADS) {
    const int64_t ab = it / BLK, a = ab / k, b = ab % k;
    const int e = (int)(it % BLK), r = e / MAX_NC, c = e % MAX_NC;
    const int32_t cam_a = cam_sorted[s + a], off_a = cam_off[cam_a], np_a = cam_off[cam_a + 1] - off_a;
    const int32_t cam_b = cam_sorted[s + b], off_b = cam_off[cam_b], np_b = cam_off[cam_b + 1] - off_b;
    const int32_t row = off_a + r, col = off_b + c;
    if (r >= np_a || c >= np_b || row > col) continue;
    const double* y = Y + (s + a) * WB + 3 * r;
    const double* w = Wblk + (s + b) * WB + 3 * c;
    atomicAdd(&Sacc[(int64_t)row * ncp + col], -(y[0] * w[0] + y[1] * w[1] + y[2] * w[2]));
  }
}

__global__ void __launch_bounds__(COV_BLOCK)
k_unc_d(int64_t n_points, const double* __restrict__ points, const double* __restrict__ Zbuf, double* __restrict__ D) {
  double acc[COV_GAUGE * (COV_GAUGE + 1) / 2];
#pragma unroll
  for (int e = 0; e < COV_GAUGE * (COV_GAUGE + 1) / 2; ++e) acc[e] = 0.0;
  for (int64_t p = (int64_t)blockIdx.x * COV_BLOCK + threadIdx.x; p < n_points; p += (int64_t)gridDim.x * COV_BLOCK) {
    double N[3][COV_GAUGE], Z[3][COV_GAUGE];
    cov_gauge_point(points[3 * p], points[3 * p + 1], points[3 * p + 2], N);
#pragma unroll
    for (int a = 0; a < 3; ++a)
#pragma unroll
      for (int j = 0; j < COV_GAUGE; ++j) Z[a][j] = Zbuf[p * (3 * COV_GAUGE) + a * COV_GAUGE + j];
    int e = 0;
#pragma unroll
    for (int j = 0; j < COV_GAUGE; ++j)
#pragma unroll
      for (int m = j; m < COV_GAUGE; ++m) acc[e++] += N[0][j] * Z[0][m] + N[1][j] * Z[1][m] + N[2][j] * Z[2][m];
  }
  int e = 0;
#pragma unroll
  for (int j = 0; j < COV_GAUGE; ++j)
#pragma unroll
    for (int m = j; m < COV_GAUGE; ++m) {
      const double v = wave_sum(acc[e++]);
      if ((threadIdx.x & 63) == 0) atomicAdd(&D[j * COV_GAUGE + m], v);
    }
}

__device__ __forceinline__ double st_entry(int row, int col, int32_t ncp, const double* __restrict__ U, const double* __restrict__ Sacc,
                                           const double* __restrict__ B, const double* __restrict__ Dinv, const int32_t* __restrict__ param_cam,
                                           const int32_t* __restrict__ param_loc) {
  double v = Sacc[(int64_t)row * ncp + col];
  if (param_cam[row] == param_cam[col]) v += U[(int64_t)param_cam[row] * (MAX_NC * MAX_NC) + param_loc[row] * MAX_NC + param_loc[col]];
#pragma unroll
  for (int j = 0; j < COV_GAUGE; ++j) {
    double s = 0.0;
#pragma unroll
    for (int m = 0; m < COV_GAUGE; ++m) s += Dinv[j * COV_GAUGE + m] * B[(int64_t)col * COV_GAUGE + m];
    v += B[(int64_t)row * COV_GAUGE + j] * s;
  }
  return v;
}

__global__ void __launch_bounds__(COV_BLOCK)
k_unc_assemble(int32_t ncp, int ldw, const double* __restrict__ U, const double* __restrict__ Sacc, const double* __restrict__ B,
               const double* __restrict__ Dinv, const int32_t* __restrict__ param_cam, const int32_t* __restrict__ param_loc,
               double* __restrict__ W, double* __restrict__ scale, int* __restrict__ flags) {
  const int64_t t = (int64_t)blockIdx.x * COV_BLOCK + threadIdx.x;
  if (t >= (int64_t)ncp * ncp) return;
  const int row = (int)(t / ncp), col = (int)(t % ncp);
  if (col < row) return;
  const double dr = st_entry(row, row, ncp, U, Sacc, B, Dinv, param_cam, param_loc);
  const double dc = st_entry(col, col, ncp, U, Sacc, B, Dinv, param_cam, param_loc);
  double sr = 1.0, sc = 1.0;
  if (dr > 0.0 && dr < 1.7e308) sr = 1.0 / sqrt(dr); else flags[F_DIAG] = 1;
  if (dc > 0.0 && dc < 1.7e308) sc = 1.0 / sqrt(dc); else flags[F_DIAG] = 1;
  const double v = (row == col ? dr : st_entry(row, col, ncp, U, Sacc, B, Dinv, param_cam, param_loc)) * sr * sc;
  W[(int64_t)row * ldw + col] = v;
  W[(int64_t)col * ldw + row] = v;
  if (row == col) scale[row] = sr;
}

__global__ void __launch_bounds__(COV_BLOCK)
k_unc_pivots(int n, int ldw, const double* __restrict__ W, int* __restrict__ flags) {
  const int j = blockIdx.x * COV_BLOCK + threadIdx.x;
  if (j >= n) return;
  const double l = W[(int64_t)j * ldw + j];
  if (!(l * l > COV_PIVOT_TINY) || !(l < 1.7e308)) flags[F_TINY] = 1;
}

__global__ void __launch_bounds__(256)
k_unc_ttt(int n, int ldw, const double* __restrict__ T, const double* __restrict__ scale, double* __restrict__ C) {
  const int bi = blockIdx.y, bj = blockIdx.x;
  if (bj < bi) return;
  const int wv = threadIdx.x >> 6, lane = threadIdx.x & 63;
  const int ti = wv >> 1, tj = wv & 1, lr = lane & 15, kq = 4 * (lane >> 4);
  const double* pa = T + (int64_t)(bi * NB + ti * 16 + lr) * ldw + kq;
  const double* pb = T + (int64_t)(bj * NB + tj * 16 + lr) * ldw + kq;
  v4f64 acc = {0.0, 0.0, 0.0, 0.0};
  for (int q0 = bj * NB; q0 < ldw; q0 += 16) {
    const double2 a0 = *reinterpret_cast<const double2*>(pa + q0), a1 = *reinterpret_cast<const double2*>(pa + q0 + 2);
    const double2 b0 = *reinterpret_cast<const double2*>(pb + q0), b1 = *reinterpret_cast<const double2*>(pb + q0 + 2);
    acc = __builtin_amdgcn_mfma_f64_16x16x4f64(a0.x, b0.x, acc, 0, 0, 0);
    acc = __builtin_amdgcn_mfma_f64_16x16x4f64(a0.y, b0.y, acc, 0, 0, 0);
    acc = __builtin_amdgcn_mfma_f64_16x16x4f64(a1.x, b1.x, acc, 0, 0, 0);
    acc = __builtin_amdgcn_mfma_f64_16x16x4f64(a1.y, b1.y, acc, 0, 0, 0);
  }
#pragma unroll
  for (int r = 0; r < 4; ++r) {
    const int gi = bi * NB + ti * 16 + (lane >> 4) + 4 * r, gj = bj * NB + tj * 16 + lr;
    if (gi < n && gj < n && gi <= gj) {
      const double v = acc[r] * scale[gi] * scale[gj];
      C[(int64_t)gi * n + gj] = v;
      C[(int64_t)gj * n + gi] = v;
    }
  }
}

__global__ void __launch_bounds__(COV_POINT_THREADS)
k_unc_point_cov(const int64_t* __restrict__ pt_start, const int32_t* __restrict__ cam_sorted, const int32_t* __restrict__ cam_off, int32_t ncp,
                const double* __restrict__ Y, const double* __restrict__ Vinv, const double* __restrict__ Zbuf, const double* __restrict__ C,
                const double* __restrict__ E, const double* __restrict__ F, double sigma0_sq, double* __restrict__ out) {
  const int64_t p = blockIdx.x;
  const int t = threadIdx.x;
  const int64_t s = pt_start[p], k = pt_start[p + 1] - s;
  constexpr int WB = 3 * MAX_NC;
  double Z[3][COV_GAUGE];
#pragma unroll
  for (int a = 0; a < 3; ++a)
#pragma unroll
    for (int j = 0; j < COV_GAUGE; ++j) Z[a][j] = Zbuf[p * (3 * COV_GAUGE) + a * COV_GAUGE + j];
  double full[3][3] = {{0.0, 0.0, 0.0}, {0.0, 0.0, 0.0}, {0.0, 0.0, 0.0}};
  for (int64_t it = t; it < k * k; it += COV_POINT_THREADS) {
    const int64_t a = it / k, b = it % k;
    const int32_t cam_a = cam_sorted[s + a], off_a = cam_off[cam_a], np_a = cam_off[cam_a + 1] - off_a;
    const int32_t cam_b = cam_sorted[s + b], off_b = cam_off[cam_b], np_b = cam_off[cam_b + 1] - off_b;
    double Yb[WB];
#pragma unroll
    for (int e = 0; e < WB; ++e) Yb[e] = Y[(s + b) * WB + e];
#pragma unroll
    for (int r = 0; r < MAX_NC; ++r) {
      if (r < np_a) {
        const double* crow = C + (int64_t)(off_a + r) * ncp + off_b;
        double t3[3] = {0.0, 0.0, 0.0};
#pragma unroll
        for (int c = 0; c < MAX_NC; ++c) {
          const double cv = c < np_b ? crow[c] : 0.0;
#pragma unroll
          for (int q = 0; q < 3; ++q) t3[q] += cv * Yb[3 * c + q];
        }
        const double* ya = Y + (s + a) * WB + 3 * r;
#pragma unroll
        for (int pp = 0; pp < 3; ++pp)
#pragma unroll
          for (int q = 0; q < 3; ++q) full[pp][q] += ya[pp] * t3[q];
      }
    }
  }
  for (int64_t a = t; a < k; a += COV_POINT_THREADS) {
    const int32_t cam_a = cam_sorted[s + a], off_a = cam_off[cam_a], np_a = cam_off[cam_a + 1] - off_a;
#pragma unroll
    for (int r = 0; r < MAX_NC; ++r) {
      if (r < np_a) {
        const double* er = E + (int64_t)(off_a + r) * COV_GAUGE;
        double t3[3] = {0.0, 0.0, 0.0};
#pragma unroll
        for (int j = 0; j < COV_GAUGE; ++j) {
          const double ev = er[j];
#pragma unroll
          for (int q = 0; q < 3; ++q) t3[q] += ev * Z[q][j];
        }
        const double* ya = Y + (s + a) * WB + 3 * r;
#pragma unroll
        for (int pp = 0; pp < 3; ++pp)
#pragma unroll
          for (int q = 0; q < 3; ++q) full[pp][q] += 2.0 * ya[pp] * t3[q];
      }
    }
  }
#pragma unroll
  for (int pp = 0; pp < 3; ++pp)
#pragma unroll
    for (int q = 0; q < 3; ++q) full[pp][q] = wave_sum(full[pp][q]);
  if (t != 0) return;
  double Vi[6], Fm[COV_GAUGE * COV_GAUGE], P[6];
#pragma unroll
  for (int e = 0; e < 6; ++e) Vi[e] = Vinv[p * 6 + e];
#pragma unroll
  for (int e = 0; e < COV_GAUGE * COV_GAUGE; ++e) Fm[e] = F[e];
  cov_point_base(Vi, Z, Fm, P);
  int e = 0;
#pragma unroll
  for (int pp = 0; pp < 3; ++pp)
#pragma unroll
    for (int q = pp; q < 3; ++q) {
      out[p * 6 + e] = sigma0_sq * (P[e] + 0.5 * (full[pp][q] + full[q][pp]));
      ++e;
    }
}

}

extern "C" int cba_parameter_covariance(const cba_cov_desc* d, int32_t device, cba_cov_out* out) {
  const char* what = "cba_parameter_covariance";
  if (!d || !out) return err(CBA_ERR_INVALID, std::string(what) + ": null argument");
  std::string msg;
  CovPlan plan;
  int rc = cov_validate(d, plan, msg);
  if (rc) return err(rc, msg);
  rc = select_device(device, what);
  if (rc) return rc;
  const int32_t n_cams = d->n_cams, ncp = plan.ncp();
  const int64_t n_obs = d->n_obs, n_points = d->n_points;
  const int nbk = (ncp + NB - 1) / NB, ldw = nbk * NB;
  std::vector<int32_t> param_cam((size_t)ncp), param_loc((size_t)ncp);
  for (int32_t c = 0; c < n_cams; ++c)
    for (int32_t r = plan.cam_off[(size_t)c]; r < plan.cam_off[(size_t)c + 1]; ++r) { param_cam[(size_t)r] = c; param_loc[(size_t)r] = r - plan.cam_off[(size_t)c]; }
  std::vector<double> cam_x((size_t)n_cams * MAX_NC, 0.0);
  for (int32_t c = 0; c < n_cams; ++c)
    for (int i = 0; i < d->cam_nparams[c]; ++i) cam_x[(size_t)c * MAX_NC + i] = d->cam_x[(size_t)c * MAX_NC + i];

  Buffers buf;
  const int32_t* dmodel = buf.in(d->cam_model, n_cams);
  const int32_t* dcam_off = buf.in(plan.cam_off.data(), n_cams + 1);
  const double* dconst = buf.in(d->cam_const, n_cams, CAM_CONST_STRIDE);
  const double* dcam_x = buf.in(cam_x.data(), n_cams, MAX_NC);
  const double* dpoints = buf.in(d->points, n_points, 3);
  const int32_t* dobs_cam = buf.in(d->obs_cam, n_obs);
  const int32_t* dobs_pt = buf.in(d->obs_pt, n_obs);
  const double* dobs_uv = buf.in(d->obs_uv, n_obs, 2);
  const int64_t* dorder = buf.in(plan.order.data(), n_obs);
  const int64_t* dpt_start = buf.in(plan.pt_start.data(), n_points + 1);
  const int32_t* dparam_cam = buf.in(param_cam.data(), ncp);
  const int32_t* dparam_loc = buf.in(param_loc.data(), ncp);
  double* dtab = buf.make<double>(n_cams, CAMTAB_DOUBLES);
  double* dWblk = buf.make<double>(n_obs, 3 * MAX_NC);
  double* dVobs = buf.make<double>(n_obs, 6);
  double* dY = buf.make<double>(n_obs, 3 * MAX_NC);
  int32_t* dcam_sorted = buf.make<int32_t>(n_obs);
  double* dVinv = buf.make<double>(n_points, 6);
  double* dZ = buf.make<double>(n_points, 3 * COV_GAUGE);
  double* dB = buf.make<double>(ncp, COV_GAUGE);
  double* dscale = buf.make<double>(ncp);
  double* dC = buf.make<double>(ncp, ncp);
  double* dXinv = buf.make<double>(nbk + 1, NB * NB);
  const size_t n_U = (size_t)n_cams * MAX_NC * MAX_NC, n_S = (size_t)ncp * ncp, n_W = ((size_t)ldw + 1) * ldw, n_T = (size_t)ldw * ldw;
  const size_t n_zero = n_U + n_S + COV_GAUGE * COV_GAUGE + 1 + n_W + n_T + N_FLAGS;
  double* dzero = buf.make<double>(n_zero);
  if (buf.status()) return buf.result(what);
  double* dW = dzero;
  double* dT = dW + n_W;
  double* dU = dT + n_T;
  double* dSacc = dU + n_U;
  double* dD = dSacc + n_S;
  double* dcost = dD + COV_GAUGE * COV_GAUGE;
  int* dflags = reinterpret_cast<int*>(dcost + 1);
  buf.check(hipMemsetAsync(dzero, 0, n_zero * sizeof(double), 0));
  if (buf.status()) return buf.result(what);

  const auto blocks = [](int64_t n) { return dim3((unsigned)((n + COV_BLOCK - 1) / COV_BLOCK)); };
  hipLaunchKernelGGL(k_unc_cam, blocks(n_cams), dim3(COV_BLOCK), 0, 0, n_cams, dmodel, dcam_off, dconst, dcam_x, dtab, dB);
  hipLaunchKernelGGL(k_unc_obs, blocks(n_obs), dim3(COV_BLOCK), 0, 0, n_obs, dorder, dobs_cam, dobs_pt, dobs_uv, (const double*)dtab, dpoints, (int)d->loss,
                     d->f_scale, dWblk, dVobs, dcam_sorted, dU, dcost);
  hipLaunchKernelGGL(k_unc_point, dim3((unsigned)n_points), dim3(COV_POINT_THREADS), 0, 0, dpt_start, (const int32_t*)dcam_sorted, dcam_off, ncp, dpoints,
                     (const double*)dWblk, (const double*)dVobs, dY, dVinv, dZ, dB, dSacc, dflags);
  const int64_t d_blocks = (n_points + COV_BLOCK - 1) / COV_BLOCK;
  hipLaunchKernelGGL(k_unc_d, dim3((unsigned)(d_blocks < 256 ? d_blocks : 256)), dim3(COV_BLOCK), 0, 0, n_points, dpoints, (const double*)dZ, dD);
  buf.check(hipGetLastError());
  std::vector<double> D(COV_GAUGE * COV_GAUGE + 1);
  std::vector<int> flags(N_FLAGS, 0);
  buf.out(D.data(), (const double*)dD, COV_GAUGE * COV_GAUGE + 1);
  buf.out(flags.data(), (const int*)dflags, N_FLAGS);
  if (buf.status()) return buf.result(what);
  if (flags[F_POINT])
    return err(CBA_ERR_NUMERIC, std::string(what) + ": point " + std::to_string(flags[F_WHICH] - 1) + ": its observations do not determine it (rays parallel or not finite)");
  const double cost = D[COV_GAUGE * COV_GAUGE];
  D.resize(COV_GAUGE * COV_GAUGE);
  for (int j = 0; j < COV_GAUGE; ++j)
    for (int m = j + 1; m < COV_GAUGE; ++m) D[(size_t)m * COV_GAUGE + j] = D[(size_t)j * COV_GAUGE + m];
  if (!std::isfinite(cost) || !cov_spd_inverse(D, COV_GAUGE))
    return err(CBA_ERR_NUMERIC, std::string(what) + ": the points do not fix the seven gauge directions (all on one line, or not finite)");
  const double sigma0_sq = 2.0 * cost / (double)plan.dof;
  const double* dDinv = buf.in(D.data(), COV_GAUGE * COV_GAUGE);
  if (buf.status()) return buf.result(what);

  hipLaunchKernelGGL(k_unc_assemble, blocks((int64_t)ncp * ncp), dim3(COV_BLOCK), 0, 0, ncp, ldw, (const double*)dU, (const double*)dSacc, (const double*)dB, dDinv,
                     dparam_cam, dparam_loc, dW, dscale, dflags);
  enqueue_chol_factor(dW, ncp, ldw, dflags, nullptr, dXinv, dT, 0);
  hipLaunchKernelGGL(k_unc_pivots, blocks(ncp), dim3(COV_BLOCK), 0, 0, (int)ncp, ldw, (const double*)dW, dflags);
  hipLaunchKernelGGL(k_unc_ttt, dim3((unsigned)nbk, (unsigned)nbk), dim3(256), 0, 0, (int)ncp, ldw, (const double*)dT, (const double*)dscale, dC);
  buf.check(hipGetLastError());
  std::vector<double> C(n_S), B((size_t)ncp * COV_GAUGE);
  buf.out(flags.data(), (const int*)dflags, N_FLAGS);
  buf.out(C.data(), (const double*)dC, ncp, ncp);
  buf.out(B.data(), (const double*)dB, ncp, COV_GAUGE);
  if (buf.status()) return buf.result(what);
  if (flags[F_DIAG] || flags[F_CHOL] || flags[F_TINY])
    return err(CBA_ERR_NUMERIC, std::string(what) + ": the reduced camera system is not positive definite beyond the gauge (a pivot is not safely positive): "
                                                    "the scene does not determine every camera parameter");
  std::vector<double> point_cov;
  if (out->point_cov) {
    std::vector<double> E, F;
    cov_gauge_terms(ncp, C.data(), B.data(), D.data(), E, F);
    const double* dE = buf.in(E.data(), ncp, COV_GAUGE);
    const double* dF = buf.in(F.data(), COV_GAUGE * COV_GAUGE);
    double* dout = buf.make<double>(n_points, 6);
    if (buf.status()) return buf.result(what);
    hipLaunchKernelGGL(k_unc_point_cov, dim3((unsigned)n_points), dim3(COV_POINT_THREADS), 0, 0, dpt_start, (const int32_t*)dcam_sorted, dcam_off, ncp,
                       (const double*)dY, (const double*)dVinv, (const double*)dZ, (const double*)dC, dE, dF, sigma0_sq, dout);
    buf.check(hipGetLastError());
    point_cov.resize((size_t)n_points * 6);
    buf.out(point_cov.data(), (const double*)dout, n_points, 6);
    if (buf.status()) return buf.result(what);
    for (double v : point_cov)
      if (!std::isfinite(v)) return err(CBA_ERR_NUMERIC, std::string(what) + ": a point covariance is not finite");
  }
  for (double v : C)
    if (!std::isfinite(v)) return err(CBA_ERR_NUMERIC, std::string(what) + ": a camera covariance is not finite");
  if (out->point_cov) std::copy(point_cov.begin(), point_cov.end(), out->point_cov);
  if (out->cam_cov_full)
    for (size_t i = 0; i < n_S; ++i) out->cam_cov_full[i] = sigma0_sq * C[i];
  if (out->cam_cov)
    for (int32_t c = 0; c < n_cams; ++c) {
      const int32_t off = plan.cam_off[(size_t)c], np = plan.cam_off[(size_t)c + 1] - off;
      for (int r = 0; r < MAX_NC; ++r)
        for (int q = 0; q < MAX_NC; ++q)
          out->cam_cov[((size_t)c * MAX_NC + r) * MAX_NC + q] = (r < np && q < np) ? sigma0_sq * C[(size_t)(off + r) * ncp + off + q] : 0.0;
    }
  if (out->sigma0_sq) *out->sigma0_sq = sigma0_sq;
  if (out->dof) *out->dof = plan.dof;
  if (out->cost) *out->cost = cost;
  return CBA_OK;
}
```

Measured before the change: 3.733 billion obs/s.

## Add look-ahead Cholesky schedule updating the next panel column early

Introduces a chol_schedule header that decodes workgroup roles for the blocked Cholesky steps. A new EARLY variant makes panel blocks also apply the update for the next column (k+1), passing intermediate results through side slots in an enlarged Xinv buffer. This shortens the critical path between consecutive step kernels and removes one trailing column per step. The diff also adds an optional deterministic fixed-order summation path in the covariance code, which is off by default. The cost is more register and shared-memory pressure in the panel kernel and more intricate indexing.

```diff
diff --git a/caliscope_amd/build.py b/caliscope_amd/build.py
--- a/caliscope_amd/build.py
+++ b/caliscope_amd/build.py
@@ -11,7 +11,7 @@
 CSRC = HERE / "csrc"
 OUT = HERE / "libcaliscope_ba.so"
 SOURCES = [CSRC / "cba_lib.hip", CSRC / "cba_solve.cpp", CSRC / "pose_lib.hip", CSRC / "scale_lib.hip", CSRC / "coverage_lib.hip", CSRC / "vertical_lib.hip", CSRC / "report_lib.hip", CSRC / "trajectory_lib.hip", CSRC / "covariance_lib.hip"]
-DEPENDS = [CSRC / "cba_kernels.h", CSRC / "schur_plan.h", CSRC / "host_plan.h", CSRC / "wg_binding.h", CSRC / "ba_math.h", CSRC / "trf_math.h", CSRC / "pnp_math.h", CSRC / "epipolar_math.h", CSRC / "intrinsic_math.h", CSRC / "frame_select_math.h", CSRC / "scale_math.h", CSRC / "coverage_math.h", CSRC / "vertical_math.h", CSRC / "report_math.h", CSRC / "trajectory_math.h", CSRC / "covariance_math.h", CSRC / "device_call.h",
+DEPENDS = [CSRC / "cba_kernels.h", CSRC / "schur_plan.h", CSRC / "chol_schedule.h", CSRC / "host_plan.h", CSRC / "wg_binding.h", CSRC / "ba_math.h", CSRC / "trf_math.h", CSRC / "pnp_math.h", CSRC / "epipolar_math.h", CSRC / "intrinsic_math.h", CSRC / "frame_select_math.h", CSRC / "scale_math.h", CSRC / "coverage_math.h", CSRC / "vertical_math.h", CSRC / "report_math.h", CSRC / "trajectory_math.h", CSRC / "covariance_math.h", CSRC / "device_call.h",
            HERE.parent / "include" / "caliscope_ba.h", HERE.parent / "include" / "caliscope_pose.h", HERE.parent / "include" / "caliscope_coverage.h", HERE.parent / "include" / "caliscope_vertical.h", HERE.parent / "include" / "caliscope_report.h", HERE.parent / "include" / "caliscope_trajectory.h", HERE.parent / "include" / "caliscope" / "uncertainty.h"]
 ARCH = "gfx950"
 
diff --git a/caliscope_amd/csrc/cba_kernels.h b/caliscope_amd/csrc/cba_kernels.h
--- a/caliscope_amd/csrc/cba_kernels.h
+++ b/caliscope_amd/csrc/cba_kernels.h
@@ -4,6 +4,7 @@
 #include "ba_math.h"
 #include "trf_math.h"
 #include "wg_binding.h"
+#include "chol_schedule.h"
 
 namespace cba {
 
@@ -2034,32 +2035,37 @@
 typedef double v4f64 __attribute__((ext_vector_type(4)));
 constexpr int CHOL_THREADS = 512;
 
+__device__ __forceinline__ v4f64 chol_rank_nb_tile(const double* __restrict__ A, int rcA, const double* __restrict__ B, int rcB, int ldw, int tile, int lane) {
+  const int ti = tile >> 1, tj = tile & 1, lr = lane & 15, kq = 4 * (lane >> 4);
+  const double* pa = A + (long)min(ti * 16 + lr, rcA - 1) * ldw + kq;
+  const double* pb = B + (long)min(tj * 16 + lr, rcB - 1) * ldw + kq;
+  double2 a[NB / 16][2], b[NB / 16][2];
+#pragma unroll
+  for (int s = 0; s < NB / 16; ++s)
+#pragma unroll
+    for (int h = 0; h < 2; ++h) {
+      a[s][h] = *reinterpret_cast<const double2*>(pa + 16 * s + 2 * h);
+      b[s][h] = *reinterpret_cast<const double2*>(pb + 16 * s + 2 * h);
+    }
+  v4f64 c = {0.0, 0.0, 0.0, 0.0};
+#pragma unroll
+  for (int s = 0; s < NB / 16; ++s)
+#pragma unroll
+    for (int h = 0; h < 2; ++h) {
+      c = __builtin_amdgcn_mfma_f64_16x16x4f64(a[s][h].x, b[s][h].x, c, 0, 0, 0);
+      c = __builtin_amdgcn_mfma_f64_16x16x4f64(a[s][h].y, b[s][h].y, c, 0, 0, 0);
+    }
+  return c;
+}
 __device__ __forceinline__ void chol_rank_nb(const double* __restrict__ A, int rcA, const double* __restrict__ B, int rcB,
                                              int ldw, double (*red)[16][17], int wv, int lane) {
   if (wv >= 4) return;
-  const int ti = wv >> 1, tj = wv & 1, lr = lane & 15, kq = 4 * (lane >> 4);
-  const double* pa = A + (long)min(ti * 16 + lr, rcA - 1) * ldw + kq;
-  const double* pb = B + (long)min(tj * 16 + lr, rcB - 1) * ldw + kq;
-  double2 a[NB / 16][2], b[NB / 16][2];
-#pragma unroll
-  for (int s = 0; s < NB / 16; ++s)
-#pragma unroll
-    for (int h = 0; h < 2; ++h) {
-      a[s][h] = *reinterpret_cast<const double2*>(pa + 16 * s + 2 * h);
-      b[s][h] = *reinterpret_cast<const double2*>(pb + 16 * s + 2 * h);
-    }
-  v4f64 c = {0.0, 0.0, 0.0, 0.0};
-#pragma unroll
-  for (int s = 0; s < NB / 16; ++s)
-#pragma unroll
-    for (int h = 0; h < 2; ++h) {
-      c = __builtin_amdgcn_mfma_f64_16x16x4f64(a[s][h].x, b[s][h].x, c, 0, 0, 0);
-      c = __builtin_amdgcn_mfma_f64_16x16x4f64(a[s][h].y, b[s][h].y, c, 0, 0, 0);
-    }
-#pragma unroll
-  for (int r = 0; r < 4; ++r) red[wv][(lane >> 4) + 4 * r][lr] = c[r];
-}
-
+  const v4f64 c = chol_rank_nb_tile(A, rcA, B, rcB, ldw, wv, lane);
+#pragma unroll
+  for (int r = 0; r < 4; ++r) red[wv][(lane >> 4) + 4 * r][lane & 15] = c[r];
+}
+
+template <bool EARLY>
 __global__ void __launch_bounds__(CHOL_THREADS)
 k_chol_step(double* __restrict__ W, int n, int ldw, int k, int* __restrict__ flags, long long* __restrict__ trace, double* __restrict__ Xinv,
             double* __restrict__ Tinv = nullptr) {
@@ -2071,12 +2077,10 @@
   const int nbk = (n + NB - 1) / NB;
   constexpr int EPT = NB * NB / CHOL_THREADS, ISTEP = CHOL_THREADS / NB;
   const int j = tid & 31, i0 = tid >> 5;
-  const int n_panel = (k < 0) ? 1 : nbk - k;
-  const int n_trailing = (k < 1) ? 0 : (nbk - k - 1) * (nbk - k) / 2;
-
-  if ((int)blockIdx.x >= n_panel + n_trailing) {
-    const int t2 = blockIdx.x - n_panel - n_trailing;
-    const int bi = k + t2 / k, bj = t2 % k, m = k - 1;
+  const CholWork wk = chol_decode<EARLY>(nbk, k, (int)blockIdx.x, Tinv != nullptr);
+
+  if (wk.role == CHOL_INVERSE) {
+    const int bi = wk.bi, bj = wk.bj, m = k - 1;
     const int ri = bi * NB, rci = min(NB, n - ri), rj = bj * NB, rcj = min(NB, n - rj);
     double* Tb = Tinv + (long)rj * ldw + ri;
     double old[EPT];
@@ -2119,10 +2123,8 @@
     return;
   }
 
-  if ((int)blockIdx.x >= n_panel) {
-    int t = blockIdx.x - n_panel, bj = k + 1;
-    while (t >= nbk - bj) { t -= nbk - bj; ++bj; }
-    const int bi = bj + 1 + t;
+  if (wk.role == CHOL_TRAILING) {
+    const int bi = wk.bi, bj = wk.bj;
     const int ri = (bi < nbk) ? bi * NB : n, rci = (bi < nbk) ? min(NB, n - ri) : 1;
     const int rj = bj * NB, rcj = min(NB, n - rj);
     const int m0 = (k - 1) * NB;
@@ -2143,16 +2145,20 @@
     return;
   }
 
-  const int b = k + 1 + blockIdx.x;
+  const int b = wk.bi;
   const int rb = (b < nbk) ? b * NB : n;
   const int rc = (b < nbk) ? min(NB, n - rb) : 1;
   const bool has_diag = b < nbk;
   double* Wb = W + (long)rb * ldw;
-  const bool stamp = trace != nullptr && blockIdx.x == 0 && tid == 0;
+  const bool stamp = trace != nullptr && wk.critical && tid == 0;
 #define CHOL_STAMP(ph) do { if (stamp) trace[(k + 1) * 8 + (ph)] = wall_clock64(); } while (0)
   CHOL_STAMP(0);
 
   double d_ij[EPT], m_ij[EPT], l_ij[EPT];
+  const bool early = EARLY && wk.early;
+  const int r1 = (k + 1) * NB, rc1 = min(NB, n - r1);
+  double* side = Xinv + (long)chol_side_slot(nbk, 0) * NB * NB;
+  const int eti = (wv >> 1) & 1, etj = wv & 1;
 #pragma unroll
   for (int h = 0; h < EPT; ++h) {
     const int i = i0 + h * ISTEP;
@@ -2169,16 +2175,44 @@
       m_ij[h] = (i < rc && j < nbp) ? Wb[(long)i * ldw + k0 + j] : 0.0;
       l_ij[h] = Xinv[(long)k * NB * NB + i * NB + j];
     }
+    double u_ij[EPT];
+    v4f64 w_e = {0.0, 0.0, 0.0, 0.0};
+    if constexpr (EARLY) {
+#pragma unroll
+      for (int h = 0; h < EPT; ++h) {
+        const int i = i0 + h * ISTEP;
+        u_ij[h] = (early && i < rc1) ? side[(long)k * NB * NB + i * NB + j] : 0.0;
+      }
+      if (early && wv >= 4) {
+#pragma unroll
+        for (int r = 0; r < 4; ++r) {
+          const int i = eti * 16 + (lane >> 4) + 4 * r, jj = etj * 16 + (lane & 15);
+          w_e[r] = (i < rc && jj < rc1) ? Wb[(long)i * ldw + r1 + jj] : 0.0;
+        }
+        if (wk.upd_terms == 2) {
+          const v4f64 c = chol_rank_nb_tile(Wb + (k0 - NB), rc, W + (long)r1 * ldw + (k0 - NB), rc1, ldw, wv - 4, lane);
+#pragma unroll
+          for (int r = 0; r < 4; ++r) w_e[r] -= c[r];
+        }
+      }
+    }
 
     CHOL_STAMP(1);
-    if (k >= 1) chol_rank_nb(Wb + (k0 - NB), rc, W + (long)k0 * ldw + (k0 - NB), nbp, ldw, sh_red, wv, lane);
-    __syncthreads();
-    CHOL_STAMP(2);
+    if constexpr (!EARLY) {
+      if (k >= 1) chol_rank_nb(Wb + (k0 - NB), rc, W + (long)k0 * ldw + (k0 - NB), nbp, ldw, sh_red, wv, lane);
+      __syncthreads();
+      CHOL_STAMP(2);
+    }
 #pragma unroll
     for (int h = 0; h < EPT; ++h) {
       const int i = i0 + h * ISTEP;
-      const double upd = (k >= 1) ? sh_red[(i >> 4) * 2 + (j >> 4)][i & 15][j & 15] : 0.0;
-      sh_U[i][j] = m_ij[h] - upd;
+      if constexpr (EARLY) {
+        sh_U[i][j] = m_ij[h];
+        if (early) sh_D[NB + i][j] = u_ij[h];
+      } else {
+        const double upd = (k >= 1) ? sh_red[(i >> 4) * 2 + (j >> 4)][i & 15][j & 15] : 0.0;
+        sh_U[i][j] = m_ij[h] - upd;
+      }
       sh_L[i][j] = l_ij[h];
     }
     __syncthreads();
@@ -2196,6 +2230,18 @@
         const int i = ti * 16 + (lane >> 4) + 4 * r, jj = tj * 16 + (lane & 15);
         sh_X[i][jj] = (jj < nbp && i < rc) ? c[r] : 0.0;
       }
+    } else if (EARLY && early) {
+      v4f64 c = {0.0, 0.0, 0.0, 0.0};
+#pragma unroll
+      for (int t = 0; t < NB / 4; ++t) {
+        const int q = 4 * t + (lane >> 4);
+        c = __builtin_amdgcn_mfma_f64_16x16x4f64(sh_D[NB + eti * 16 + (lane & 15)][q], sh_L[etj * 16 + (lane & 15)][q], c, 0, 0, 0);
+      }
+#pragma unroll
+      for (int r = 0; r < 4; ++r) {
+        const int i = eti * 16 + (lane >> 4) + 4 * r, jj = etj * 16 + (lane & 15);
+        sh_D[i][jj] = (i < rc1) ? c[r] : 0.0;
+      }
     }
     __syncthreads();
 #pragma unroll
@@ -2204,6 +2250,24 @@
       if (i < rc && j < nbp) Wb[(long)i * ldw + k0 + j] = sh_X[i][j];
     }
     CHOL_STAMP(4);
+    if (EARLY && early && wv >= 4) {
+      v4f64 c = {0.0, 0.0, 0.0, 0.0};
+#pragma unroll
+      for (int t = 0; t < NB / 4; ++t) {
+        const int q = 16 * (t >> 2) + 4 * (lane >> 4) + (t & 3);
+        c = __builtin_amdgcn_mfma_f64_16x16x4f64(sh_X[eti * 16 + (lane & 15)][q], sh_D[etj * 16 + (lane & 15)][q], c, 0, 0, 0);
+      }
+      double* next_u = (wk.side_write >= 0) ? side + (long)wk.side_write * NB * NB : nullptr;
+#pragma unroll
+      for (int r = 0; r < 4; ++r) {
+        const int i = eti * 16 + (lane >> 4) + 4 * r, jj = etj * 16 + (lane & 15);
+        if (i < rc && jj < rc1) {
+          const double v = w_e[r] - c[r];
+          Wb[(long)i * ldw + r1 + jj] = v;
+          if (next_u) next_u[i * NB + jj] = v;
+        }
+      }
+    }
     if (!has_diag) return;
     if (wv < 4) {
       const int ti = wv >> 1, tj = wv & 1;
@@ -2231,7 +2295,13 @@
   }
   __syncthreads();
   CHOL_STAMP(5);
-  if (tid < WAVE) chol_factor_block(sh_D, rc, flags);
+  if (tid < WAVE) {
+    chol_factor_block(sh_D, rc, flags);
+  } else if (EARLY && k < 0 && wk.side_write >= 0) {
+    const int live = min(NB, n - NB);
+    for (int e = tid - WAVE; e < NB * NB; e += CHOL_THREADS - WAVE)
+      if (e / NB < live) side[e] = W[(long)(NB + e / NB) * ldw + e % NB];
+  }
   __syncthreads();
   chol_factor_store(sh_D, rc, Wb + rb, ldw, Xinv + (long)(k + 1) * NB * NB, tid, CHOL_THREADS, Tinv ? Tinv + (long)rb * ldw + rb : nullptr);
   CHOL_STAMP(6);
diff --git a/caliscope_amd/csrc/cba_lib.hip b/caliscope_amd/csrc/cba_lib.hip
--- a/caliscope_amd/csrc/cba_lib.hip
+++ b/caliscope_amd/csrc/cba_lib.hip
@@ -104,6 +104,7 @@
   double* tri = nullptr;
   double* Xinv = nullptr;
   double* Tinv = nullptr;
+  bool chol_early = true;
   bool fuse_reg_finalize = true;
   double* scal = nullptr;
   double* xbuf = nullptr;
@@ -1126,7 +1127,7 @@
   TRYS(dev_alloc(p, &p->S, (size_t)ncp * ncp)); p->ldw = (ncp + 3) & ~3;
   if (p->want_chol_trace) TRYS(dev_alloc(p, &p->chol_trace, (size_t)((ncp + NB - 1) / NB + 2) * 8));
   TRYS(dev_alloc(p, &p->Lbuf, (size_t)(ncp + 1) * p->ldw));
-  TRYS(dev_alloc(p, &p->Xinv, (size_t)((ncp + NB - 1) / NB + 1) * NB * NB));
+  TRYS(dev_alloc(p, &p->Xinv, (size_t)chol_xinv_blocks((ncp + NB - 1) / NB) * NB * NB));
   TRYS(dev_zeros(p, &p->Tinv, (size_t)ncp * p->ldw));
   TRYS(dev_alloc(p, &p->rhs, (size_t)p->lay.ncp_pad));
   TRYS(dev_zeros(p, &p->scal, 64)); TRYS(dev_zeros(p, &p->flags, 8)); TRYS(dev_alloc(p, &p->xbuf, 128));
@@ -1180,6 +1181,7 @@
   p->C = d->n_cams; p->P = d->n_points; p->N = d->n_obs;
   p->loss = d->loss; p->f_scale = d->f_scale;
   if (const char* e = std::getenv("CBA_REG_FINALIZE")) p->fuse_reg_finalize = e[0] != '0';
+  if (const char* e = std::getenv("CBA_CHOL_EARLY")) p->chol_early = e[0] != '0';
   if (const char* e = std::getenv("CBA_SPEC_SKIP")) p->spec_skip = e[0] != '0';
   if (const char* e = std::getenv("CBA_SMALL_SOLVE")) p->small_solve_on = e[0] != '0';
 #ifdef CBA_PROFILING
@@ -1587,20 +1589,24 @@
 
 namespace cba {
 __attribute__((visibility("hidden"))) void enqueue_chol_factor(double* W, int n, int ldw, int* flags, long long* trace, double* Xinv, double* Tinv,
-                                                               hipStream_t stream) {
+                                                               bool early, hipStream_t stream) {
   const int nbk = (n + NB - 1) / NB;
   for (int k = -1; k < nbk; ++k) {
-    const int n_panel = k < 0 ? 1 : nbk - k;
-    const int x = nbk - k - 1, n_trailing = k < 1 ? 0 : x * (x + 1) / 2;
-    const int n_inverse = (k >= 1) ? (nbk - k) * k : 0;
-    hipLaunchKernelGGL(k_chol_step, dim3(n_panel + n_trailing + n_inverse), dim3(CHOL_THREADS), 0, stream, W, n, ldw, k, flags, trace, Xinv, Tinv);
-  }
+    if (early)
+      hipLaunchKernelGGL(k_chol_step<true>, dim3(chol_counts<true>(nbk, k, Tinv != nullptr).total()), dim3(CHOL_THREADS), 0, stream, W, n, ldw, k, flags, trace, Xinv, Tinv);
+    else
+      hipLaunchKernelGGL(k_chol_step<false>, dim3(chol_counts<false>(nbk, k, Tinv != nullptr).total()), dim3(CHOL_THREADS), 0, stream, W, n, ldw, k, flags, trace, Xinv, Tinv);
+  }
+}
+__attribute__((visibility("hidden"))) bool chol_early_from_env() {
+  const char* e = std::getenv("CBA_CHOL_EARLY");
+  return !(e && e[0] == '0');
 }
 }
 
 static int enqueue_cholesky(cba_problem* p) {
   const int n = p->ncp, nbk = (n + NB - 1) / NB;
-  enqueue_chol_factor(p->Lbuf, n, p->ldw, p->flags, p->chol_trace, p->Xinv, p->Tinv, p->stream);
+  enqueue_chol_factor(p->Lbuf, n, p->ldw, p->flags, p->chol_trace, p->Xinv, p->Tinv, p->chol_early, p->stream);
   hipLaunchKernelGGL(k_chol_apply, dim3(nbk), dim3(APPLY_THREADS), (size_t)n * 8, p->stream, (const double*)p->Tinv, (const double*)p->Lbuf, n, p->ldw, p->s);
   return CBA_OK;
 }
@@ -1617,8 +1623,12 @@
     HIPCHK(hipStreamSynchronize(p->stream));
     for (int s = 0; s <= nbk; ++s) {
       fprintf(stderr, "chol step %2d:", s - 1);
+      int last = 0;
       for (int ph = 1; ph < 7; ++ph)
-        if (h[s * 8 + ph] && h[s * 8 + ph - 1]) fprintf(stderr, " ph%d %6.2f us", ph, (h[s * 8 + ph] - h[s * 8 + ph - 1]) * 0.01); else if (h[s * 8 + ph]) fprintf(stderr, " ph%d (%6.2f)", ph, (h[s * 8 + ph] - h[s * 8]) * 0.01);
+        if (h[s * 8 + ph]) {
+          if (h[s * 8 + last]) fprintf(stderr, " ph%d %6.2f us", ph, (h[s * 8 + ph] - h[s * 8 + last]) * 0.01); else fprintf(stderr, " ph%d (      )", ph);
+          last = ph;
+        }
       if (s < nbk && h[(s + 1) * 8] && h[s * 8]) fprintf(stderr, "  | to next step start %6.2f us", (h[(s + 1) * 8] - h[s * 8]) * 0.01);
       fprintf(stderr, "\n");
     }
diff --git a/caliscope_amd/csrc/chol_schedule.h b/caliscope_amd/csrc/chol_schedule.h
--- /dev/null
+++ b/caliscope_amd/csrc/chol_schedule.h
@@ -0,0 +1,136 @@
+#pragma once
+
+#if defined(__HIPCC__) || defined(__CUDACC__)
+#define CHOL_HD __host__ __device__
+#else
+#define CHOL_HD
+#endif
+
+namespace cba {
+
+enum CholRole : int { CHOL_FACTOR0 = 0, CHOL_PANEL = 1, CHOL_TRAILING = 2, CHOL_INVERSE = 3 };
+
+CHOL_HD inline int chol_xinv_blocks(int nbk) { return 2 * (nbk + 1); }
+CHOL_HD inline int chol_side_slot(int nbk, int s) { return nbk + 1 + s; }
+
+struct CholCounts {
+  int panel, trailing, inverse;
+  CHOL_HD int total() const { return panel + trailing + inverse; }
+};
+
+template <bool EARLY>
+CHOL_HD inline int chol_first_trailing_column(int k) { return k + (EARLY ? 2 : 1); }
+
+template <bool EARLY>
+CHOL_HD inline CholCounts chol_counts(int nbk, int k, bool with_inverse) {
+  CholCounts c;
+  c.panel = (k < 0) ? 1 : nbk - k;
+  const int x = nbk - chol_first_trailing_column<EARLY>(k);
+  c.trailing = (k < 1 || x < 1) ? 0 : x * (x + 1) / 2;
+  c.inverse = (with_inverse && k >= 1) ? (nbk - k) * k : 0;
+  return c;
+}
+
+struct CholWork {
+  int role, bi, bj;
+  bool critical, early;
+  int upd_col, upd_first, upd_terms, side_write;
+};
+
+template <bool EARLY>
+CHOL_HD inline CholWork chol_decode(int nbk, int k, int wg, bool with_inverse) {
+  const CholCounts cnt = chol_counts<EARLY>(nbk, k, with_inverse);
+  CholWork w;
+  w.critical = false; w.early = false;
+  w.upd_col = -1; w.upd_first = 0; w.upd_terms = 0; w.side_write = -1;
+  if (k < 0) {
+    w.role = CHOL_FACTOR0; w.bi = 0; w.bj = 0; w.critical = true;
+    if (EARLY && nbk >= 2) w.side_write = 0;
+    return w;
+  }
+  if (wg < cnt.panel) {
+    w.role = CHOL_PANEL; w.bi = k + 1 + wg; w.bj = k;
+    w.critical = wg == 0;
+    if (EARLY) {
+      if (w.bi >= k + 2 && k + 1 < nbk) {
+        w.early = true;
+        w.upd_col = k + 1; w.upd_first = (k >= 1) ? k - 1 : k; w.upd_terms = (k >= 1) ? 2 : 1;
+        if (w.bi == k + 2 && k + 2 < nbk) w.side_write = k + 1;
+      }
+    } else if (k >= 1) {
+      w.upd_col = k; w.upd_first = k - 1; w.upd_terms = 1;
+    }
+    return w;
+  }
+  if (wg < cnt.panel + cnt.trailing) {
+    int t = wg - cnt.panel, bj = chol_first_trailing_column<EARLY>(k);
+    while (t >= nbk - bj) { t -= nbk - bj; ++bj; }
+    w.role = CHOL_TRAILING; w.bi = bj + 1 + t; w.bj = bj;
+    w.upd_col = bj; w.upd_first = k - 1; w.upd_terms = 1;
+    return w;
+  }
+  const int t2 = wg - cnt.panel - cnt.trailing;
+  w.role = CHOL_INVERSE; w.bi = k + t2 / k; w.bj = t2 % k;
+  return w;
+}
+
+enum CholBuf : int { CHOL_W = 0, CHOL_XINV = 1, CHOL_SIDE = 2, CHOL_T = 3 };
+struct CholRef {
+  int buf, i, j;
+};
+
+template <bool EARLY, class F>
+inline void chol_for_each_access(int nbk, int k, int wg, bool with_inverse, F&& f) {
+  const CholWork w = chol_decode<EARLY>(nbk, k, wg, with_inverse);
+  const auto rd = [&](int buf, int i, int j) { f(CholRef{buf, i, j}, false); };
+  const auto wr = [&](int buf, int i, int j) { f(CholRef{buf, i, j}, true); };
+  if (w.role == CHOL_FACTOR0) {
+    rd(CHOL_W, 0, 0); wr(CHOL_W, 0, 0); wr(CHOL_XINV, 0, 0);
+    if (with_inverse) wr(CHOL_T, 0, 0);
+    if (w.side_write >= 0) { rd(CHOL_W, 1, 0); wr(CHOL_SIDE, w.side_write, 0); }
+    return;
+  }
+  if (w.role == CHOL_PANEL) {
+    const int b = w.bi;
+    const bool has_diag = b < nbk;
+    rd(CHOL_W, b, k); rd(CHOL_XINV, k, 0); wr(CHOL_W, b, k);
+    if (has_diag) { rd(CHOL_W, b, b); wr(CHOL_W, b, b); }
+    if (w.critical && has_diag) { wr(CHOL_XINV, k + 1, 0); if (with_inverse) wr(CHOL_T, b, b); }
+    if (w.upd_col >= 0) {
+      for (int m = w.upd_first; m < k; ++m) { rd(CHOL_W, b, m); rd(CHOL_W, w.upd_col, m); }
+      if (w.early) { rd(CHOL_SIDE, k, 0); rd(CHOL_W, b, w.upd_col); wr(CHOL_W, b, w.upd_col); }
+      if (w.side_write >= 0) wr(CHOL_SIDE, w.side_write, 0);
+    }
+    return;
+  }
+  if (w.role == CHOL_TRAILING) {
+    rd(CHOL_W, w.bi, w.bj); rd(CHOL_W, w.bi, k - 1); rd(CHOL_W, w.bj, k - 1); wr(CHOL_W, w.bi, w.bj);
+    return;
+  }
+  const int m = k - 1;
+  if (m != w.bj) rd(CHOL_T, w.bj, w.bi);
+  rd(CHOL_T, w.bj, m); rd(CHOL_W, w.bi, m);
+  if (w.bi == k) rd(CHOL_XINV, k, 0);
+  wr(CHOL_T, w.bj, w.bi);
+}
+
+enum CholAct : int { CHOL_ACT_APPLY = 0, CHOL_ACT_SOLVE = 1, CHOL_ACT_FACTOR = 2 };
+
+template <bool EARLY, class F>
+inline void chol_for_each_action(int nbk, int k, int wg, bool with_inverse, F&& f) {
+  const CholWork w = chol_decode<EARLY>(nbk, k, wg, with_inverse);
+  if (w.role == CHOL_FACTOR0) { f(CHOL_ACT_FACTOR, 0, 0, 0); return; }
+  if (w.role == CHOL_INVERSE) return;
+  if (w.role == CHOL_TRAILING) { f(CHOL_ACT_APPLY, w.bi, w.bj, w.upd_first); return; }
+  const int b = w.bi;
+  if (!w.early && w.upd_col >= 0) f(CHOL_ACT_APPLY, b, k, w.upd_first);
+  f(CHOL_ACT_SOLVE, b, k, k);
+  if (w.early)
+    for (int t = 0; t < w.upd_terms; ++t) f(CHOL_ACT_APPLY, b, w.upd_col, w.upd_first + t);
+  if (b < nbk) {
+    f(CHOL_ACT_APPLY, b, b, k);
+    if (w.critical) f(CHOL_ACT_FACTOR, b, b, b);
+  }
+}
+
+}
diff --git a/caliscope_amd/csrc/covariance_lib.hip b/caliscope_amd/csrc/covariance_lib.hip
--- a/caliscope_amd/csrc/covariance_lib.hip
+++ b/caliscope_amd/csrc/covariance_lib.hip
@@ -2,16 +2,19 @@
 
 #include <algorithm>
 #include <cmath>
+#include <cstdlib>
 #include <string>
 #include <vector>
 
 #include "ba_math.h"
 #include "covariance_math.h"
 #include "device_call.h"
+#include "chol_schedule.h"
 
 namespace cba {
 __attribute__((visibility("hidden"))) void enqueue_chol_factor(double* W, int n, int ldw, int* flags, long long* trace, double* Xinv, double* Tinv,
-                                                               hipStream_t stream);
+                                                               bool early, hipStream_t stream);
+__attribute__((visibility("hidden"))) bool chol_early_from_env();
 }
 
 using namespace cba;
@@ -55,7 +58,8 @@
 __global__ void __launch_bounds__(COV_BLOCK)
 k_unc_obs(int64_t n_obs, const int64_t* __restrict__ order, const int32_t* __restrict__ obs_cam, const int32_t* __restrict__ obs_pt,
           const double* __restrict__ obs_uv, const double* __restrict__ tab, const double* __restrict__ points, int loss, double f_scale,
-          double* __restrict__ Wblk, double* __restrict__ Vobs, int32_t* __restrict__ cam_sorted, double* __restrict__ U, double* __restrict__ cost) {
+          double* __restrict__ Wblk, double* __restrict__ Vobs, int32_t* __restrict__ cam_sorted, double* __restrict__ U, double* __restrict__ cost,
+          bool fixed_order) {
   const int64_t i = (int64_t)blockIdx.x * COV_BLOCK + threadIdx.x;
   double rho = 0.0;
   if (i < n_obs) {
@@ -73,6 +77,7 @@
 #pragma unroll
     for (int e = 0; e < 6; ++e) Vobs[i * 6 + e] = Vo[e];
     cam_sorted[i] = cam;
+    if (fixed_order) return;
     const bool nine = c.nparams == 9.0;
     double* Uc = U + (int64_t)cam * (MAX_NC * MAX_NC);
 #pragma unroll
@@ -81,14 +86,52 @@
       for (int q = r; q < MAX_NC; ++q)
         if (q < 6 || nine) atomicAdd(&Uc[r * MAX_NC + q], A[0][r] * A[0][q] + A[1][r] * A[1][q]);
   }
+  if (fixed_order) return;
   rho = wave_sum(rho);
   if ((threadIdx.x & 63) == 0 && rho != 0.0) atomicAdd(cost, 0.5 * rho);
+}
+
+__global__ void __launch_bounds__(64)
+k_unc_cam_sums(int64_t n_obs, const int64_t* __restrict__ order, const int32_t* __restrict__ obs_pt, const double* __restrict__ obs_uv,
+               const double* __restrict__ tab, const double* __restrict__ points, int loss, double f_scale, const int32_t* __restrict__ cam_sorted,
+               double* __restrict__ U, double* __restrict__ cam_cost) {
+  const int32_t cam = blockIdx.x;
+  const CamTab& c = reinterpret_cast<const CamTab*>(tab)[cam];
+  const bool nine = c.nparams == 9.0;
+  double acc[MAX_NC * (MAX_NC + 1) / 2], rho = 0.0;
+#pragma unroll
+  for (int e = 0; e < MAX_NC * (MAX_NC + 1) / 2; ++e) acc[e] = 0.0;
+  for (int64_t i = threadIdx.x; i < n_obs; i += 64) {
+    if (cam_sorted[i] != cam) continue;
+    const int64_t o = order[i], p = obs_pt[o];
+    const double X[3] = {points[3 * p], points[3 * p + 1], points[3 * p + 2]};
+    const double uv[2] = {obs_uv[2 * o], obs_uv[2 * o + 1]};
+    double A[2][MAX_NC], B[2][3];
+    rho += cov_obs_jacobian(c, X, uv, loss, f_scale, A, B);
+    int e = 0;
+#pragma unroll
+    for (int r = 0; r < MAX_NC; ++r)
+#pragma unroll
+      for (int q = r; q < MAX_NC; ++q) acc[e++] += A[0][r] * A[0][q] + A[1][r] * A[1][q];
+  }
+  double* Uc = U + (int64_t)cam * (MAX_NC * MAX_NC);
+  int e = 0;
+#pragma unroll
+  for (int r = 0; r < MAX_NC; ++r)
+#pragma unroll
+    for (int q = r; q < MAX_NC; ++q) {
+      const double v = wave_sum(acc[e++]);
+      if (threadIdx.x == 0 && (q < 6 || nine)) Uc[r * MAX_NC + q] += v;
+    }
+  rho = wave_sum(rho);
+  if (threadIdx.x == 0) cam_cost[cam] = 0.5 * rho;
 }
 
 __global__ void __launch_bounds__(COV_POINT_THREADS)
 k_unc_point(const int64_t* __restrict__ pt_start, const int32_t* __restrict__ cam_sorted, const int32_t* __restrict__ cam_off, int32_t ncp,
             const double* __restrict__ points, const double* __restrict__ Wblk, const double* __restrict__ Vobs, double* __restrict__ Y,
-            double* __restrict__ Vinv, double* __restrict__ Zbuf, double* __restrict__ B, double* __restrict__ Sacc, int* __restrict__ flags) {
+            double* __restrict__ Vinv, double* __restrict__ Zbuf, double* __restrict__ B, double* __restrict__ Sacc, int* __restrict__ flags,
+            bool fixed_order) {
   __shared__ double sh_vi[9], sh_z[3 * COV_GAUGE];
   const int64_t p = blockIdx.x;
   const int t = threadIdx.x;
@@ -127,6 +170,7 @@
     Y[(s + a) * WB + e] = w[0] * sh_vi[q] + w[1] * sh_vi[3 + q] + w[2] * sh_vi[6 + q];
   }
   __syncthreads();
+  if (fixed_order) return;
   for (int64_t it = t; it < k * (MAX_NC * COV_GAUGE); it += COV_POINT_THREADS) {
     const int64_t a = it / (MAX_NC * COV_GAUGE);
     const int e = (int)(it % (MAX_NC * COV_GAUGE)), r = e / COV_GAUGE, j = e % COV_GAUGE;
@@ -149,8 +193,42 @@
   }
 }
 
+constexpr int COV_ROWS_THREADS = 192;
+__global__ void __launch_bounds__(COV_ROWS_THREADS)
+k_unc_rows(int64_t n_points, const int64_t* __restrict__ pt_start, const int32_t* __restrict__ cam_sorted, const int32_t* __restrict__ cam_off, int32_t ncp,
+           const double* __restrict__ Wblk, const double* __restrict__ Y, const double* __restrict__ Zbuf, double* __restrict__ B, double* __restrict__ Sacc) {
+  constexpr int WB = 3 * MAX_NC;
+  const int32_t cam = blockIdx.x, off_a = cam_off[cam], np_a = cam_off[cam + 1] - off_a;
+  const int t = threadIdx.x;
+  const bool b_role = t < MAX_NC * COV_GAUGE, s_role = t >= 64 && t < 64 + MAX_NC * MAX_NC;
+  const int e = b_role ? t : t - 64;
+  const int r = b_role ? e / COV_GAUGE : e / MAX_NC, c = b_role ? e % COV_GAUGE : e % MAX_NC;
+  if (!(b_role || s_role) || r >= np_a) return;
+  for (int64_t p = 0; p < n_points; ++p) {
+    const int64_t s = pt_start[p], k = pt_start[p + 1] - s;
+    for (int64_t a = 0; a < k; ++a) {
+      if (cam_sorted[s + a] != cam) continue;
+      if (b_role) {
+        const double* w = Wblk + (s + a) * WB + 3 * r;
+        const double* z = Zbuf + p * (3 * COV_GAUGE);
+        B[(int64_t)(off_a + r) * COV_GAUGE + c] += -(w[0] * z[c] + w[1] * z[COV_GAUGE + c] + w[2] * z[2 * COV_GAUGE + c]);
+        continue;
+      }
+      const double* y = Y + (s + a) * WB + 3 * r;
+      for (int64_t b = 0; b < k; ++b) {
+        const int32_t cam_b = cam_sorted[s + b], off_b = cam_off[cam_b], np_b = cam_off[cam_b + 1] - off_b;
+        const int32_t row = off_a + r, col = off_b + c;
+        if (c >= np_b || row > col) continue;
+        const double* w = Wblk + (s + b) * WB + 3 * c;
+        Sacc[(int64_t)row * ncp + col] += -(y[0] * w[0] + y[1] * w[1] + y[2] * w[2]);
+      }
+    }
+  }
+}
+
+constexpr int COV_D_BLOCKS = 256;
 __global__ void __launch_bounds__(COV_BLOCK)
-k_unc_d(int64_t n_points, const double* __restrict__ points, const double* __restrict__ Zbuf, double* __restrict__ D) {
+k_unc_d(int64_t n_points, const double* __restrict__ points, const double* __restrict__ Zbuf, double* __restrict__ D, double* __restrict__ rows) {
   double acc[COV_GAUGE * (COV_GAUGE + 1) / 2];
 #pragma unroll
   for (int e = 0; e < COV_GAUGE * (COV_GAUGE + 1) / 2; ++e) acc[e] = 0.0;
@@ -172,9 +250,28 @@
   for (int j = 0; j < COV_GAUGE; ++j)
 #pragma unroll
     for (int m = j; m < COV_GAUGE; ++m) {
-      const double v = wave_sum(acc[e++]);
-      if ((threadIdx.x & 63) == 0) atomicAdd(&D[j * COV_GAUGE + m], v);
-    }
+      const double v = wave_sum(acc[e]);
+      if ((threadIdx.x & 63) == 0) {
+        if (rows) rows[((int64_t)blockIdx.x * (COV_BLOCK / 64) + (threadIdx.x >> 6)) * 28 + e] = v; else atomicAdd(&D[j * COV_GAUGE + m], v);
+      }
+      ++e;
+    }
+}
+
+__global__ void __launch_bounds__(64)
+k_unc_fixed_sums(const double* __restrict__ rows, int n_rows, const double* __restrict__ cam_cost, int32_t n_cams, double* __restrict__ D, double* __restrict__ cost) {
+  const int e = threadIdx.x;
+  if (e < 28) {
+    double v = 0.0;
+    for (int i = 0; i < n_rows; ++i) v += rows[(int64_t)i * 28 + e];
+    int j = 0, rest = e;
+    while (rest >= COV_GAUGE - j) { rest -= COV_GAUGE - j; ++j; }
+    D[j * COV_GAUGE + j + rest] = v;
+  } else if (e == 28) {
+    double v = 0.0;
+    for (int32_t c = 0; c < n_cams; ++c) v += cam_cost[c];
+    *cost = v;
+  }
 }
 
 __device__ __forceinline__ double st_entry(int row, int col, int32_t ncp, const double* __restrict__ U, const double* __restrict__ Sacc,
@@ -373,7 +470,13 @@
   double* dB = buf.make<double>(ncp, COV_GAUGE);
   double* dscale = buf.make<double>(ncp);
   double* dC = buf.make<double>(ncp, ncp);
-  double* dXinv = buf.make<double>(nbk + 1, NB * NB);
+  const char* det_env = std::getenv("CBA_DETERMINISTIC");
+  const bool fixed_order = det_env && det_env[0] != '\0' && !(det_env[0] == '0' && det_env[1] == '\0');
+  const int64_t d_blocks_all = (n_points + COV_BLOCK - 1) / COV_BLOCK;
+  const int d_grid = (int)(d_blocks_all < COV_D_BLOCKS ? d_blocks_all : COV_D_BLOCKS), d_rows = d_grid * (COV_BLOCK / 64);
+  double* dD_rows = fixed_order ? buf.make<double>(d_rows, 28) : nullptr;
+  double* dcam_cost = fixed_order ? buf.make<double>(n_cams) : nullptr;
+  double* dXinv = buf.make<double>(chol_xinv_blocks(nbk), NB * NB);
   const size_t n_U = (size_t)n_cams * MAX_NC * MAX_NC, n_S = (size_t)ncp * ncp, n_W = ((size_t)ldw + 1) * ldw, n_T = (size_t)ldw * ldw;
   const size_t n_zero = n_U + n_S + COV_GAUGE * COV_GAUGE + 1 + n_W + n_T + N_FLAGS;
   double* dzero = buf.make<double>(n_zero);
@@ -391,11 +494,18 @@
   const auto blocks = [](int64_t n) { return dim3((unsigned)((n + COV_BLOCK - 1) / COV_BLOCK)); };
   hipLaunchKernelGGL(k_unc_cam, blocks(n_cams), dim3(COV_BLOCK), 0, 0, n_cams, dmodel, dcam_off, dconst, dcam_x, dtab, dB);
   hipLaunchKernelGGL(k_unc_obs, blocks(n_obs), dim3(COV_BLOCK), 0, 0, n_obs, dorder, dobs_cam, dobs_pt, dobs_uv, (const double*)dtab, dpoints, (int)d->loss,
-                     d->f_scale, dWblk, dVobs, dcam_sorted, dU, dcost);
+                     d->f_scale, dWblk, dVobs, dcam_sorted, dU, dcost, fixed_order);
+  if (fixed_order)
+    hipLaunchKernelGGL(k_unc_cam_sums, dim3((unsigned)n_cams), dim3(64), 0, 0, n_obs, dorder, dobs_pt, dobs_uv, (const double*)dtab, dpoints, (int)d->loss, d->f_scale,
+                       (const int32_t*)dcam_sorted, dU, dcam_cost);
   hipLaunchKernelGGL(k_unc_point, dim3((unsigned)n_points), dim3(COV_POINT_THREADS), 0, 0, dpt_start, (const int32_t*)dcam_sorted, dcam_off, ncp, dpoints,
-                     (const double*)dWblk, (const double*)dVobs, dY, dVinv, dZ, dB, dSacc, dflags);
-  const int64_t d_blocks = (n_points + COV_BLOCK - 1) / COV_BLOCK;
-  hipLaunchKernelGGL(k_unc_d, dim3((unsigned)(d_blocks < 256 ? d_blocks : 256)), dim3(COV_BLOCK), 0, 0, n_points, dpoints, (const double*)dZ, dD);
+                     (const double*)dWblk, (const double*)dVobs, dY, dVinv, dZ, dB, dSacc, dflags, fixed_order);
+  if (fixed_order)
+    hipLaunchKernelGGL(k_unc_rows, dim3((unsigned)n_cams), dim3(COV_ROWS_THREADS), 0, 0, n_points, dpt_start, (const int32_t*)dcam_sorted, dcam_off, ncp,
+                       (const double*)dWblk, (const double*)dY, (const double*)dZ, dB, dSacc);
+  hipLaunchKernelGGL(k_unc_d, dim3((unsigned)d_grid), dim3(COV_BLOCK), 0, 0, n_points, dpoints, (const double*)dZ, dD, dD_rows);
+  if (fixed_order)
+    hipLaunchKernelGGL(k_unc_fixed_sums, dim3(1), dim3(64), 0, 0, (const double*)dD_rows, d_rows, (const double*)dcam_cost, n_cams, dD, dcost);
   buf.check(hipGetLastError());
   std::vector<double> D(COV_GAUGE * COV_GAUGE + 1);
   std::vector<int> flags(N_FLAGS, 0);
@@ -416,7 +526,7 @@
 
   hipLaunchKernelGGL(k_unc_assemble, blocks((int64_t)ncp * ncp), dim3(COV_BLOCK), 0, 0, ncp, ldw, (const double*)dU, (const double*)dSacc, (const double*)dB, dDinv,
                      dparam_cam, dparam_loc, dW, dscale, dflags);
-  enqueue_chol_factor(dW, ncp, ldw, dflags, nullptr, dXinv, dT, 0);
+  enqueue_chol_factor(dW, ncp, ldw, dflags, nullptr, dXinv, dT, chol_early_from_env(), 0);
   hipLaunchKernelGGL(k_unc_pivots, blocks(ncp), dim3(COV_BLOCK), 0, 0, (int)ncp, ldw, (const double*)dW, dflags);
   hipLaunchKernelGGL(k_unc_ttt, dim3((unsigned)nbk, (unsigned)nbk), dim3(256), 0, 0, (int)ncp, ldw, (const double*)dT, (const double*)dscale, dC);
   buf.check(hipGetLastError());
```

Measured after the change: 3.776 billion obs/s (median of 6 runs). 1.01x the previous value.
